# rapidsai/cudf

Measured on AMD Instinct MI355X. Metric: rows/sec + achieved HBM GB/s: 1e9-row int64 sort & hash-join, 1/2/4/8 GPU, higher is better.
Workload: dtype int64; 1 GPU; 1e+09-row int64 radix sort (cudf::sort, keys only); rows_per_gpu=1000000000, algo=0, parallelism=1 GPU

## Files before the change

cudf_amd/csrc/gx_common.hpp:

```cpp
#pragma once

#include <hip/hip_runtime.h>

#include <atomic>
#include <stdint.h>

#include "../../include/cudf_amd/gx.h"
#include "gx_lds_book.hpp"

#define GX_WAVE 64

#define GX_HIP_TRY(expr)                           \
  do {                                             \
    const int _e = (int)(expr);                    \
    if (_e != (int)hipSuccess) return _e;          \
  } while (0)

#define GX_LAUNCH_CHECK()                          \
  do {                                             \
    hipError_t _e = hipGetLastError();             \
    if (_e != hipSuccess) return (int)_e;          \
  } while (0)

namespace gx {
// ... 47 lines not shown
template <typename Kernel, typename... Args>
inline int launch_lds(const Device& dev, Kernel kernel, dim3 grid, dim3 block, size_t lds_bytes, hipStream_t s, Args&&... args)
{
  GX_HIP_TRY(lds_book().ensure(reinterpret_cast<const void*>(kernel), dev.id, (int)lds_bytes, set_max_dynamic_lds));
  hipLaunchKernelGGL(kernel, grid, block, lds_bytes, s, static_cast<Args&&>(args)...);
  return 0;
}
inline int max_resident_wgs(const Device& dev, const void* kernel, int block, size_t lds_bytes, int* wgs)
{
  GX_HIP_TRY(lds_book().ensure(kernel, dev.id, (int)lds_bytes, set_max_dynamic_lds));
  GX_HIP_TRY(hipOccupancyMaxActiveBlocksPerMultiprocessor(wgs, kernel, block, lds_bytes));
  if (*wgs < 1) *wgs = 1;
  return 0;
}

__device__ __forceinline__ unsigned lane_id()
{
  return __builtin_amdgcn_mbcnt_hi(~0u, __builtin_amdgcn_mbcnt_lo(~0u, 0u));
}
__device__ __forceinline__ uint64_t lanemask_lt() { return (1ull << lane_id()) - 1ull; }
__device__ __forceinline__ uint64_t ballot(bool p) { return __builtin_amdgcn_ballot_w64(p); }

template <typename T, typename F>
__device__ __forceinline__ T shfl_words(T v, F f)
{
  static_assert(sizeof(T) % 4 == 0, "shuffle payload must be a multiple of 4 bytes");
  uint32_t w[sizeof(T) / 4];
  __builtin_memcpy(w, &v, sizeof(T));
#pragma unroll
  for (unsigned k = 0; k < sizeof(T) / 4; ++k) w[k] = f(w[k]);
  T r;
  __builtin_memcpy(&r, w, sizeof(T));
  return r;
}
template <typename T>
__device__ __forceinline__ T shfl_up(T v, unsigned delta)
{
  return shfl_words(v, [delta](uint32_t x) { return (uint32_t)__shfl_up((int)x, delta, GX_WAVE); });
}
template <typename T>
__device__ __forceinline__ T shfl(T v, int src)
{
  return shfl_words(v, [src](uint32_t x) { return (uint32_t)__shfl((int)x, src, GX_WAVE); });
}
template <typename T>
__device__ __forceinline__ T shfl_xor(T v, int m)
{
  return shfl_words(v, [m](uint32_t x) { return (uint32_t)__shfl_xor((int)x, m, GX_WAVE); });
}

template <int NBITS>
__device__ __forceinline__ void match_rank(uint32_t d, bool live, uint64_t active, uint32_t& lower, uint32_t& count)
{
  uint32_t m_lo = (uint32_t)active, m_hi = (uint32_t)(active >> 32);
#pragma unroll
  for (int b = 0; b < NBITS; ++b) {
    const int beta   = __builtin_amdgcn_sbfe(d, b, 1);
    const uint64_t v = ballot(live && beta != 0);
    m_lo             = __builtin_amdgcn_bitop3_b32(m_lo, (uint32_t)v, (uint32_t)beta, 0x90);
    m_hi             = __builtin_amdgcn_bitop3_b32(m_hi, (uint32_t)(v >> 32), (uint32_t)beta, 0x90);
  }
  lower = __builtin_amdgcn_mbcnt_hi(m_hi, __builtin_amdgcn_mbcnt_lo(m_lo, 0u));
  count = (uint32_t)__builtin_popcount(m_lo) + (uint32_t)__builtin_popcount(m_hi);
}

template <int NBITS>
__device__ __forceinline__ uint32_t lds_rank_few(uint32_t* counters, uint32_t d, bool live)
{
  const uint64_t active = ballot(live);
  uint32_t m_lo = (uint32_t)active, m_hi = (uint32_t)(active >> 32);
#pragma unroll
  for (int b = 0; b < NBITS; ++b) {
    const int beta   = __builtin_amdgcn_sbfe(d, b, 1);
    const uint64_t v = ballot(live && beta != 0);
    m_lo             = __builtin_amdgcn_bitop3_b32(m_lo, (uint32_t)v, (uint32_t)beta, 0x90);
    m_hi             = __builtin_amdgcn_bitop3_b32(m_hi, (uint32_t)(v >> 32), (uint32_t)beta, 0x90);
  }
  const uint32_t lower = __builtin_amdgcn_mbcnt_hi(m_hi, __builtin_amdgcn_mbcnt_lo(m_lo, 0u));
  const uint32_t count = (uint32_t)__builtin_popcount(m_lo) + (uint32_t)__builtin_popcount(m_hi);
  const uint64_t m     = ((uint64_t)m_hi << 32) | m_lo;
  const int leader     = m ? __builtin_ctzll(m) : (int)lane_id();
  uint32_t base        = 0;
  if (live && lower == 0) base = atomicAdd(&counters[d], count);
  base = (uint32_t)__builtin_amdgcn_ds_bpermute(leader << 2, (int)base);
  return live ? base + lower : 0u;
}

__device__ __forceinline__ void match_rank8(uint32_t d, bool live, uint64_t active, uint32_t& lower, uint32_t& count)
{
  match_rank<8>(d, live, active, lower, count);
}

template <int M>
__device__ __forceinline__ uint32_t lane_xor32(uint32_t v)
{
  if constexpr (M == 1) return (uint32_t)__builtin_amdgcn_update_dpp(0, (int)v, 0xB1, 0xF, 0xF, false);
  else if constexpr (M == 2) return (uint32_t)__builtin_amdgcn_update_dpp(0, (int)v, 0x4E, 0xF, 0xF, false);
  else if constexpr (M == 3) return (uint32_t)__builtin_amdgcn_update_dpp(0, (int)v, 0x1B, 0xF, 0xF, false);
  else if constexpr (M == 7) return (uint32_t)__builtin_amdgcn_update_dpp(0, (int)v, 0x141, 0xF, 0xF, false);
  else if constexpr (M == 15) return (uint32_t)__builtin_amdgcn_update_dpp(0, (int)v, 0x140, 0xF, 0xF, false);
  else return (uint32_t)__builtin_amdgcn_ds_bpermute((int)((lane_id() ^ (unsigned)M) << 2), (int)v);
}
template <int M>
__device__ __forceinline__ uint64_t lane_xor64(uint64_t v)
{
  return ((uint64_t)lane_xor32<M>((uint32_t)(v >> 32)) << 32) | lane_xor32<M>((uint32_t)v);
}
template <int M, int LOWBIT>
__device__ __forceinline__ void cmpx(uint64_t& k)
{
  const uint64_t o   = lane_xor64<M>(k);
  const bool keepmin = (lane_id() & (unsigned)LOWBIT) == 0;
  k                  = ((k < o) == keepmin) ? k : o;
}
__device__ __forceinline__ void wave_bitonic64(uint64_t& k)
{
  cmpx<1, 1>(k);
  cmpx<3, 2>(k); cmpx<1, 1>(k);
  cmpx<7, 4>(k); cmpx<2, 2>(k); cmpx<1, 1>(k);
  cmpx<15, 8>(k); cmpx<4, 4>(k); cmpx<2, 2>(k); cmpx<1, 1>(k);
  cmpx<31, 16>(k); cmpx<8, 8>(k); cmpx<4, 4>(k); cmpx<2, 2>(k); cmpx<1, 1>(k);
  cmpx<63, 32>(k); cmpx<16, 16>(k); cmpx<8, 8>(k); cmpx<4, 4>(k); cmpx<2, 2>(k); cmpx<1, 1>(k);
}
__device__ __forceinline__ void wave_halfclean64(uint64_t& k)
{
  cmpx<32, 32>(k); cmpx<16, 16>(k); cmpx<8, 8>(k); cmpx<4, 4>(k); cmpx<2, 2>(k); cmpx<1, 1>(k);
}
__device__ __forceinline__ void wave_bitonic128(uint64_t& k0, uint64_t& k1)
{
  wave_bitonic64(k0);
  wave_bitonic64(k1);
  const uint64_t o1 = lane_xor64<63>(k1), o0 = lane_xor64<63>(k0);
  k0 = k0 < o1 ? k0 : o1;
  k1 = k1 < o0 ? o0 : k1;
  wave_halfclean64(k0);
  wave_halfclean64(k1);
}

__device__ __forceinline__ uint32_t lds_rank(uint32_t* counters, uint32_t d, bool live)
{
  const uint64_t act = ballot(live);
  if (act == 0) return 0;
  const int leader    = __builtin_ctzll(act);
  const uint32_t dl   = shfl(d, leader);
  const uint64_t same = ballot(live && d == dl);
  if (same == act || __builtin_popcountll(same) >= 8) {
    uint32_t base = 0;
    if ((int)lane_id() == leader) base = atomicAdd(&counters[dl], (uint32_t)__builtin_popcountll(same));
    base = shfl(base, leader);
    if (live && d == dl) return base + (uint32_t)__builtin_popcountll(same & lanemask_lt());
    return live ? atomicAdd(&counters[d], 1u) : 0u;
  }
  return live ? atomicAdd(&counters[d], 1u) : 0u;
}

struct SumOp {
  template <typename T>
  __device__ __forceinline__ T operator()(T a, T b) const { return a + b; }
};
struct MinOp {
  template <typename T>
  __device__ __forceinline__ T operator()(T a, T b) const { return b < a ? b : a; }
};
struct MaxOp {
  template <typename T>
  __device__ __forceinline__ T operator()(T a, T b) const { return a < b ? b : a; }
};
struct ProdOp {
  template <typename T>
  __device__ __forceinline__ T operator()(T a, T b) const { return a * b; }
};

template <int CTRL, int RM, typename T>
__device__ __forceinline__ T dpp_take(T v)
{
  return shfl_words(v, [](uint32_t x) { return (uint32_t)__builtin_amdgcn_update_dpp((int)x, (int)x, CTRL, RM, 0xF, false); });
}
template <int SRC, typename T>
__device__ __forceinline__ T read_lane(T v)
{
  return shfl_words(v, [](uint32_t x) { return (uint32_t)__builtin_amdgcn_readlane((int)x, SRC); });
}
template <typename T, typename Op>
__device__ __forceinline__ T wave_inclusive_scan(T v, Op op)
{
  const unsigned l = lane_id();
  { const T o = dpp_take<0x111, 0xF>(v); if ((l & 15u) >= 1u) v = op(o, v); }
  { const T o = dpp_take<0x112, 0xF>(v); if ((l & 15u) >= 2u) v = op(o, v); }
  { const T o = dpp_take<0x114, 0xF>(v); if ((l & 15u) >= 4u) v = op(o, v); }
  { const T o = dpp_take<0x118, 0xF>(v); if ((l & 15u) >= 8u) v = op(o, v); }
  { const T o = dpp_take<0x142, 0xA>(v); if (l & 16u) v = op(o, v); }
  { const T o = dpp_take<0x143, 0xC>(v); if (l >= 32u) v = op(o, v); }
  return v;
}

template <typename T, typename Op>
__device__ __forceinline__ T wave_reduce(T v, Op op)
{
#pragma unroll
  for (int d = GX_WAVE / 2; d >= 1; d >>= 1) v = op(v, shfl_xor(v, d));
  return v;
}

template <int BT, typename T, typename Op>
__device__ __forceinline__ T block_exclusive_scan(T v, T identity, Op op, T* lds, T* total)
{
  constexpr int NW = BT / GX_WAVE;
  const unsigned l = lane_id();
  const unsigned w = threadIdx.x / GX_WAVE;
  T inc            = wave_inclusive_scan(v, op);
  if (l == GX_WAVE - 1) lds[w] = inc;
  __syncthreads();
  if (w == 0) {
    T x = (l < NW) ? lds[l] : identity;
    T s = wave_inclusive_scan(x, op);
    if (l < NW) lds[l] = s;
  }
  __syncthreads();
  T wave_prefix = (w == 0) ? identity : lds[w - 1];
  T exc         = shfl_up(inc, 1);
  if (l == 0) exc = identity;
  if (total) *total = lds[NW - 1];
  T r = op(wave_prefix, exc);
  __syncthreads();
  return r;
}

__device__ __forceinline__ uint64_t dpp_wave_shl1_u64(uint64_t v, uint64_t fill)
{
  const int lo = __builtin_amdgcn_update_dpp((int)(uint32_t)fill, (int)(uint32_t)v, 0x130, 0xF, 0xF, false);
  const int hi = __builtin_amdgcn_update_dpp((int)(uint32_t)(fill >> 32), (int)(uint32_t)(v >> 32), 0x130, 0xF, 0xF, false);
  return ((uint64_t)(uint32_t)hi << 32) | (uint32_t)lo;
}
__device__ __forceinline__ uint64_t dpp_wave_shr1_u64(uint64_t v, uint64_t fill)
{
  const int lo = __builtin_amdgcn_update_dpp((int)(uint32_t)fill, (int)(uint32_t)v, 0x138, 0xF, 0xF, false);
  const int hi = __builtin_amdgcn_update_dpp((int)(uint32_t)(fill >> 32), (int)(uint32_t)(v >> 32), 0x138, 0xF, 0xF, false);
  return ((uint64_t)(uint32_t)hi << 32) | (uint32_t)lo;
}
__device__ __forceinline__ bool wave_split_sort(uint64_t* keys, uint32_t cnt, uint32_t* cw ,
                                                int sh, uint64_t& k0, uint64_t& k1)
{
  const unsigned lane = lane_id();
  const uint32_t e0 = 2 * lane, e1 = 2 * lane + 1;
  k0 = e0 < cnt ? keys[e0] : ~0ull;
  k1 = e1 < cnt ? keys[e1] : ~0ull;
  uint4* cw4  = reinterpret_cast<uint4*>(cw);
  cw4[lane]   = make_uint4(0u, 0u, 0u, 0u);
  const uint32_t b0 = (uint32_t)(k0 >> sh) & 0xFFu, b1 = (uint32_t)(k1 >> sh) & 0xFFu;
  const uint32_t r0 = e0 < cnt ? atomicAdd(&cw[b0], 1u) : 0u;
  const uint32_t r1 = e1 < cnt ? atomicAdd(&cw[b1], 1u) : 0u;
  uint4 c = cw4[lane];
  uint32_t mx = c.x > c.y ? c.x : c.y;
  mx          = c.z > mx ? c.z : mx;
  mx          = c.w > mx ? c.w : mx;
  if (ballot(mx > 4u) != 0) return false;
  const uint32_t sum = c.x + c.y + c.z + c.w;
  const uint32_t inc = wave_inclusive_scan(sum, SumOp());
  uint32_t run       = inc - sum;
  uint4 st;
  st.x = run; run += c.x;
  st.y = run; run += c.y;
  st.z = run; run += c.z;
  st.w = run;
  cw4[lane] = st;
  if (e0 < cnt) keys[cw[b0] + r0] = k0;
  if (e1 < cnt) keys[cw[b1] + r1] = k1;
  k0 = e0 < cnt ? keys[e0] : ~0ull;
  k1 = e1 < cnt ? keys[e1] : ~0ull;
#pragma unroll
  for (int ph = 0; ph < 2; ++ph) {
    {
      const bool sw     = k1 < k0;
      const uint64_t lo = sw ? k1 : k0, hi = sw ? k0 : k1;
      k0 = lo;
      k1 = hi;
    }
    {
      const uint64_t nxt = dpp_wave_shl1_u64(k0, ~0ull);
      const uint64_t prv = dpp_wave_shr1_u64(k1, 0ull);
      k1                 = nxt < k1 ? nxt : k1;
      k0                 = prv > k0 ? prv : k0;
    }
  }
  return true;
}

__device__ __forceinline__ uint32_t wave_inclusive_sum_dpp(uint32_t v)
{
  v += (uint32_t)__builtin_amdgcn_update_dpp(0, (int)v, 0x111, 0xF, 0xF, false);
  v += (uint32_t)__builtin_amdgcn_update_dpp(0, (int)v, 0x112, 0xF, 0xF, false);
  v += (uint32_t)__builtin_amdgcn_update_dpp(0, (int)v, 0x114, 0xF, 0xF, false);
  v += (uint32_t)__builtin_amdgcn_update_dpp(0, (int)v, 0x118, 0xF, 0xF, false);
  v += (uint32_t)__builtin_amdgcn_update_dpp(0, (int)v, 0x142, 0xA, 0xF, false);
  v += (uint32_t)__builtin_amdgcn_update_dpp(0, (int)v, 0x143, 0xC, 0xF, false);
  return v;
}

__device__ __forceinline__ unsigned wave_split_sort_x2(uint64_t* keysA, uint32_t cntA, uint64_t* keysB, uint32_t cntB,
                                                       uint32_t* cw , int sh, uint64_t& a0,
                                                       uint64_t& a1, uint64_t& b0, uint64_t& b1)
{
  const unsigned lane = lane_id();
  const uint32_t e0 = 2 * lane, e1 = 2 * lane + 1;
  uint32_t* cwA = cw;
  uint32_t* cwB = cw + 128;
// ... 233 lines not shown
```

cudf_amd/csrc/gx_sort.hip:

```cpp
#include "gx_common.hpp"
#include <cstdlib>
#include <type_traits>
#include <vector>
#include "gx_scan.hpp"

namespace gx {
namespace sort {

constexpr int BINS       = 256;
constexpr int MAX_PASSES = 8;
constexpr int BT         = 512;
constexpr int NW         = BT / GX_WAVE;
constexpr int NRANGE     = 8;

constexpr int CS_MAXBITS = 15;
constexpr int NB2MAX     = 1024;
constexpr int NB9        = 512;

struct HybridPlan {
  int32_t attempt;
  int32_t ok;
  int32_t shift0;
  int32_t shift2, bits2;
  int32_t nlocal;
// ... 700 lines not shown
#pragma unroll
          for (int k = 0; k < LBW; ++k) {
            const int64_t q = p - k;
            v[k]            = (q >= 0) ? load_agent_u64(&a.status[q * BINS + tid]) : pack_status(2u, epoch, 0u);
          }
#pragma unroll
          for (int k = 0; k < LBW; ++k) {
            if (!done) {
              unsigned long long x = v[k];
              uint32_t spins       = 0;
              unsigned long long spin_t0 = 0;
              while ((x >> 62) == 0 || ((unsigned)(x >> 32) & 0xFFu) != epoch) {
                if (spin_guard(spins, spin_t0, plan, a.spin_ticks)) {
                  x = pack_status(2u, epoch, 0u);
                  break;
                }
                __builtin_amdgcn_s_sleep(2);
                x = load_agent_u64(&a.status[(p - k) * BINS + tid]);
              }
              prefix += (uint32_t)x;
              if ((x >> 62) == 2u) done = true;
            }
          }
          p -= LBW;
        }
        if (tile != a.inject_tile) store_agent_u64(&a.status[tile * BINS + tid], pack_status(2u, epoch, prefix + pub_count));
      }
      gbase = plan->gbin[pass][tid] + prefix;
    } else {
      gbase = a.tile_off[(int64_t)tid * a_ntiles + tile];
    }
    s_gdelta[tid] = gbase - bin_start;
  }
  __syncthreads();

#pragma unroll
  for (int j = 0; j < KPT; ++j) {
    const int i = j * BT + (int)tid;
    if (i < nvalid) {
      const KeyT k       = s_keys[i];
      const uint32_t d   = (uint32_t)(to_sortable<KeyT, KIND>(k, desc_mask) >> shift) & 0xFFu;
      const uint32_t dst = s_gdelta[d] + (uint32_t)i;
      kout[dst]          = k;
      if (HAS_VAL) vout[dst] = s_vals[i];
    }
  }
  if (MULTI) __syncthreads();
  }
}

template <typename KeyT, int KIND, int KPT>
__global__ void __launch_bounds__(BT) k_tile_hist(PassArgs a, uint32_t* tile_hist)
{
  constexpr int TILE = BT * KPT;
  __shared__ uint32_t s_hist[BINS];
  SortPlan* plan = a.plan;
  const int pass = a.pass;
  if (plan->pass_skip[pass]) return;
  const KeyT* kin      = static_cast<const KeyT*>(a.kbuf[plan->pass_src[pass]]);
  const KeyT desc_mask = (KeyT)a.desc_mask;
  const int shift      = pass * 8;
  const unsigned tid   = threadIdx.x;
  if (tid < BINS) s_hist[tid] = 0;
  __syncthreads();
  const int64_t tile = xcd_swizzle(blockIdx.x, gridDim.x);
  const int64_t base = tile * TILE;
  const int nvalid   = (int)((a.n - base < (int64_t)TILE) ? (a.n - base) : (int64_t)TILE);
  const unsigned lane = lane_id();
#pragma unroll
  for (int j = 0; j < KPT; ++j) {
    const int i = j * BT + (int)tid;
    if (i < nvalid) {
      const uint32_t d      = (uint32_t)(to_sortable<KeyT, KIND>(kin[base + i], desc_mask) >> shift) & 0xFFu;
      const uint64_t active = ballot(true);
      const uint32_t d0     = __builtin_amdgcn_readfirstlane(d);
      if (ballot(d == d0) == active) {
        if ((int)lane == __builtin_ctzll(active)) atomicAdd(&s_hist[d0], (uint32_t)__builtin_popcountll(active));
      } else {
        atomicAdd(&s_hist[d], 1u);
      }
    }
  }
  __syncthreads();
  if (tid < BINS) tile_hist[(int64_t)tid * a.ntiles + tile] = s_hist[tid];
}

template <typename KeyT, bool HAS_VAL>
__global__ void __launch_bounds__(256) k_finalize_copy(PassArgs a)
{
  if (a.plan->num_active != 0) return;
  const bool mode_b    = a.plan->hy.lsd_mode != 0;
  const KeyT* kin      = static_cast<const KeyT*>(mode_b ? a.kbufB[0] : a.kbuf[0]);
  KeyT* kout           = static_cast<KeyT*>(mode_b ? a.kbufB[1] : a.kbuf[1]);
  const int64_t a_n    = mode_b ? (int64_t)a.plan->hy.lsd_n : a.n;
  const int64_t stride = (int64_t)gridDim.x * blockDim.x;
  for (int64_t i = (int64_t)blockIdx.x * blockDim.x + threadIdx.x; i < a_n; i += stride) {
    kout[i] = kin[i];
    if (HAS_VAL) a.vbuf[1][i] = a.vbuf[0] ? a.vbuf[0][i] : (uint32_t)i;
  }
}

template <typename KeyT, bool HAS_VAL>
__global__ void __launch_bounds__(256) k_reverse_nan_block(KeyT* keys, uint32_t* vals, int64_t n)
{
  constexpr KeyT SIGN = KeyT(1) << (sizeof(KeyT) * 8 - 1);
  constexpr KeyT EXP  = (sizeof(KeyT) == 8) ? KeyT(0x7FF0000000000000ull) : KeyT(0x7F800000u);
  __shared__ long long s_cnt;
  if (threadIdx.x == 0) {
    int64_t lo = 0, hi = n;
    while (lo < hi) {
      const int64_t mid = lo + (hi - lo) / 2;
      if ((keys[mid] & KeyT(~SIGN)) > EXP) lo = mid + 1; else hi = mid;
    }
    s_cnt = lo;
  }
  __syncthreads();
  const int64_t cnt    = s_cnt;
  const int64_t half   = cnt / 2;
  const int64_t stride = (int64_t)gridDim.x * blockDim.x;
  for (int64_t i = (int64_t)blockIdx.x * blockDim.x + threadIdx.x; i < half; i += stride) {
    const int64_t j = cnt - 1 - i;
    const KeyT a = keys[i], b = keys[j];
    keys[i] = b;
    keys[j] = a;
    if (HAS_VAL) {
      const uint32_t va = vals[i], vb2 = vals[j];
      vals[i] = vb2;
      vals[j] = va;
    }
  }
}

__device__ __forceinline__ unsigned xcc_id() { return __builtin_amdgcn_s_getreg(20 | (0 << 6) | (3 << 11)) & 7u; }

struct MsdArgs {
  const void* in;
  void* out;
  const uint32_t* vin;
  uint32_t* vout;
  SortPlan* plan;
  unsigned long long* status;
  const uint32_t* base;
  uint32_t* cellcount;
  uint32_t cellcap;
  int64_t n;
  int level;
  int exp;
  uint64_t desc_mask;
  unsigned long long spin_ticks = 0;
  long long inject_tile         = -1;
};

template <typename KeyT, int KIND, bool HAS_VAL, int KPT, int LBW, int NBL>
__global__ void __launch_bounds__(BT, (KPT <= 8 ? 8 : (KPT <= 12 ? 6 : 4))) k_msd_pass(MsdArgs a)
{
  constexpr int TILE = BT * KPT;
  constexpr int NB   = 1 << NBL;
  static_assert(NB <= BT, "one thread per bin");
  constexpr bool STABLE = KIND == K_FLOAT || HAS_VAL;
  constexpr int WROWS   = STABLE ? NW : 2;
  extern __shared__ __attribute__((aligned(16))) char smem[];
  KeyT* s_keys       = reinterpret_cast<KeyT*>(smem);
  uint32_t* s_vals   = reinterpret_cast<uint32_t*>(smem + (size_t)TILE * sizeof(KeyT));
  constexpr bool HIST16 = STABLE && HAS_VAL && NBL == 9;
  using HistT           = typename std::conditional<HIST16, uint16_t, uint32_t>::type;
  uint32_t* s_whist  = s_vals + (HAS_VAL ? TILE : 0);
  HistT* s_whist16   = reinterpret_cast<HistT*>(s_whist);
  uint32_t* s_gdelta = s_whist + (HIST16 ? WROWS * NB / 2 : WROWS * NB);
  uint32_t* s_limit  = s_gdelta + NB;
  uint32_t* s_scan   = s_limit + NB;
  uint32_t* s_misc   = s_scan + 16;

  SortPlan* plan = a.plan;
  HybridPlan& hy = plan->hy;
  const int lvl  = a.level;
  if (!hy.attempt || plan->hf.state == 3) return;
  const KeyT* kin      = static_cast<const KeyT*>(a.in);
  KeyT* kout           = static_cast<KeyT*>(a.out);
  const uint32_t* vin  = a.vin;
  uint32_t* vout       = a.vout;
  const KeyT desc_mask = (KeyT)a.desc_mask;
  const uint32_t dmask = lvl == 0 ? 0xFFu : ((1u << hy.bits2) - 1u);
  const Digit0 dig     = lvl == 0 ? digit0_of(hy, (int)(8 * sizeof(KeyT))) : Digit0{hy.shift2, 0, dmask, 0u};
  const int nseg       = lvl == 0 ? NRANGE : BINS;
  const unsigned tid   = threadIdx.x;
  const unsigned lane  = lane_id();
  const unsigned w     = tid / GX_WAVE;
  const unsigned epoch = 9u + (unsigned)lvl;

  if (tid == 0) {
    const unsigned x = ((a.exp & 1) && lvl == 1) ? 0u : ((a.exp & 2) ? (blockIdx.x % NRANGE) : xcc_id());
    uint32_t g       = 0xFFFFFFFFu;
    for (int i = 0; i < NRANGE; ++i) {
      const unsigned y   = (x + i) % NRANGE;
      const uint32_t ntl = hy.list_tile0[lvl][y + 1] - hy.list_tile0[lvl][y];
      if (ntl == 0) continue;
      const uint32_t t = atomicAdd(&plan->cnt.ctr[lvl][y].v, 1u);
      if (t < ntl) {
        g = hy.list_tile0[lvl][y] + t;
        break;
      }
    }
    s_misc[0] = g;
  }
  __syncthreads();
  {
    const uint32_t g = s_misc[0];
    if (g != 0xFFFFFFFFu && (int)tid < nseg) {
      const uint32_t lo = hy.seg_tile0[lvl][tid], hi = hy.seg_tile0[lvl][tid + 1];
      if (lo <= g && g < hi) {
        s_misc[1] = tid;
        s_misc[2] = g - lo;
      }
    }
  }
  __syncthreads();
  const uint32_t gtile = s_misc[0];
  if (gtile == 0xFFFFFFFFu) return;
  const uint32_t seg   = s_misc[1];
  const uint32_t jt    = s_misc[2];
  const int64_t base   = (int64_t)hy.seg_start[lvl][seg] + (int64_t)jt * TILE;
  const int64_t remain = (int64_t)hy.seg_count[lvl][seg] - (int64_t)jt * TILE;
  const int nvalid     = (int)(remain < (int64_t)TILE ? remain : (int64_t)TILE);
  const uint32_t l1cap  = lvl == 1 ? cell_cap(hy, seg) : 0u;
  const uint32_t l1base = lvl == 1 ? cell_slot(hy, seg, 0u) : 0u;

  KeyT key[KPT];
  uint32_t val[HAS_VAL ? KPT : 1];
  const int wbase = (int)w * (KPT * GX_WAVE) + (int)lane;
  if (nvalid == TILE) {
#pragma unroll
    for (int j = 0; j < KPT; ++j) key[j] = kin[base + wbase + j * GX_WAVE];
  } else {
#pragma unroll
    for (int j = 0; j < KPT; ++j) {
      const int idx = wbase + j * GX_WAVE;
      key[j]        = (idx < nvalid) ? kin[base + idx] : KeyT(0);
    }
  }
  if (HAS_VAL) {
#pragma unroll
    for (int j = 0; j < KPT; ++j) {
      const int idx = wbase + j * GX_WAVE;
      val[j]        = (idx < nvalid) ? (vin ? vin[base + idx] : (uint32_t)(base + idx)) : 0u;
    }
  }
  HistT* my_hist = s_whist16 + w * NB;
  uint32_t packed[KPT];
  uint32_t tile_count = 0;
  if (STABLE) {
#pragma unroll
    for (int k = 0; k < NB / ((HIST16 ? 2 : 1) * GX_WAVE); ++k) reinterpret_cast<uint32_t*>(my_hist)[lane + k * GX_WAVE] = 0;
#pragma unroll
    for (int j = 0; j < KPT; ++j) {
      const int idx = wbase + j * GX_WAVE;
      uint32_t d    = dig(to_sortable<KeyT, KIND>(key[j], desc_mask));
      if (idx >= nvalid) d = NB - 1;
      uint32_t lower, cnt;
      match_rank<NBL>(d, true, ~0ull, lower, cnt);
      const uint32_t prev = my_hist[d];
      if (lower == 0) my_hist[d] = (HistT)(prev + cnt);
      packed[j] = (d << 16) | (prev + lower);
    }
    __syncthreads();
    if (tid < NB) {
      uint32_t sum = 0;
#pragma unroll
      for (int w2 = 0; w2 < NW; ++w2) {
        const uint32_t c         = s_whist16[w2 * NB + tid];
        s_whist16[w2 * NB + tid] = (HistT)sum;
        sum += c;
      }
      tile_count = sum;
    }
  } else {
    if (tid < NB) s_whist[tid] = 0;
    __syncthreads();
#pragma unroll
    for (int j = 0; j < KPT; ++j) {
      const int idx    = wbase + j * GX_WAVE;
      const uint32_t d = dig(to_sortable<KeyT, KIND>(key[j], desc_mask));
      const uint32_t r = lds_rank(s_whist, d, idx < nvalid);
      packed[j]        = (d << 16) | r;
    }
    __syncthreads();
    if (tid < NB) tile_count = s_whist[tid];
  }
  uint32_t pub_count = tile_count;
  if (STABLE && tid == NB - 1) pub_count -= (uint32_t)(TILE - nvalid);
  if (tid < NB) {
    if ((long long)gtile != a.inject_tile) store_agent_u64(&a.status[(int64_t)gtile * NB + tid], pack_status(jt == 0 ? 2u : 1u, epoch, pub_count));
  }
  const uint32_t bin_start = block_exclusive_scan<BT>(tile_count, 0u, SumOp(), s_scan, (uint32_t*)nullptr);
  if (tid < NB) {
    if (STABLE) {
#pragma unroll
      for (int w2 = 0; w2 < NW; ++w2) s_whist16[w2 * NB + tid] = (HistT)(s_whist16[w2 * NB + tid] + bin_start);
    } else {
      s_whist[NB + tid] = bin_start;
    }
  }
  __syncthreads();

#pragma unroll
  for (int j = 0; j < KPT; ++j) {
    const uint32_t d = packed[j] >> 16;
    if (STABLE) {
      const uint32_t pos = (uint32_t)my_hist[d] + (packed[j] & 0xFFFFu);
      s_keys[pos]        = key[j];
      if (HAS_VAL) s_vals[pos] = val[j];
    } else if (wbase + j * GX_WAVE < nvalid) {
      s_keys[s_whist[NB + d] + (packed[j] & 0xFFFFu)] = key[j];
    }
  }

  if (tid < NB) {
    uint32_t prefix = 0;
    if (jt > 0) {
      int64_t p = (int64_t)gtile - 1;
      bool done = false;
      while (!done) {
        unsigned long long v[LBW];
#pragma unroll
        for (int k = 0; k < LBW; ++k) {
          const int64_t q = p - k;
          v[k]            = (q >= 0) ? load_agent_u64(&a.status[q * NB + tid]) : pack_status(2u, epoch, 0u);
        }
#pragma unroll
        for (int k = 0; k < LBW; ++k) {
          if (!done) {
            unsigned long long x = v[k];
            uint32_t spins       = 0;
            unsigned long long spin_t0 = 0;
            while ((x >> 62) == 0 || ((unsigned)(x >> 32) & 0xFFu) != epoch) {
              if (spin_guard(spins, spin_t0, a.plan, a.spin_ticks)) {
                x = pack_status(2u, epoch, 0u);
                break;
              }
              __builtin_amdgcn_s_sleep(2);
              x = load_agent_u64(&a.status[(p - k) * NB + tid]);
            }
            prefix += (uint32_t)x;
            if ((x >> 62) == 2u) done = true;
          }
        }
        p -= LBW;
      }
      if ((long long)gtile != a.inject_tile) store_agent_u64(&a.status[(int64_t)gtile * NB + tid], pack_status(2u, epoch, prefix + pub_count));
    }
    uint32_t gb, lim = 0xFFFFFFFFu;
    if (lvl == 0) {
      gb = a.base[seg * NB2MAX + tid];
    } else {
      const bool live = tid < (1u << hy.bits2);
      const uint32_t cellcap = l1cap;
      gb              = live ? l1base + tid * l1cap : 0u;
      lim             = live ? gb + cellcap : 0u;
      if (live) {
        if (prefix + pub_count > cellcap && !__hip_atomic_load(&hy.overflow, __ATOMIC_RELAXED, __HIP_MEMORY_SCOPE_AGENT))
          atomicExch(&hy.overflow, 1);
        if (gtile + 1 == hy.seg_tile0[1][seg + 1]) a.cellcount[seg * NB2MAX + tid] = prefix + pub_count;
      }
    }
    s_limit[tid]  = lim;
    s_gdelta[tid] = gb + prefix - bin_start;
  }
  __syncthreads();

#pragma unroll
  for (int j = 0; j < KPT; ++j) {
    const int i = j * BT + (int)tid;
    if (i < nvalid) {
      const KeyT k       = s_keys[i];
      const uint32_t d   = dig(to_sortable<KeyT, KIND>(k, desc_mask));
      const uint32_t dst = s_gdelta[d] + (uint32_t)i;
      if (dst < s_limit[d]) {
        kout[dst] = k;
        if (HAS_VAL) vout[dst] = s_vals[i];
      }
    }
  }
}

__global__ void __launch_bounds__(GX_WAVE) k_plan2(SortPlan* plan, uint32_t* __restrict__ cellcount,
                                                   uint32_t* __restrict__ cellstart, int npass, int cursor_path)
{
  HybridPlan& hy = plan->hy;
  if (!hy.attempt || (plan->hf.state == 3) != (cursor_path != 0)) return;
  constexpr int PER    = NB2MAX / GX_WAVE;
  const int b          = blockIdx.x;
  const unsigned lane  = lane_id();
  const uint32_t start = hy.gbin0[b];
  const uint32_t count = hy.hist0[b];
  const int nb2        = 1 << hy.bits2;
  const bool eqb = cursor_path && plan->sp.on && plan->sp.eq[b];
  const bool nrb = cursor_path && plan->sp.on && sp_narrow(plan->sp, (uint32_t)b, hy.bits2);
  uint32_t c[PER], sum = 0, mx = 0;
#pragma unroll
  for (int k = 0; k < PER; ++k) {
    const int d2 = (int)lane * PER + k;
    c[k]         = d2 < nb2 ? cellcount[b * NB2MAX + d2] : 0u;
    sum += c[k];
    if (eqb) {
      if (d2 == 0) cellcount[b * NB2MAX] = 0u;
      c[k] = 0u;
    }
    if (nrb && d2 < nb2) cellcount[b * NB2MAX + d2] = 0u;
    if (!nrb) mx = c[k] > mx ? c[k] : mx;
  }
  const uint32_t inc = wave_inclusive_sum_dpp(sum);
  uint32_t run       = start + inc - sum;
#pragma unroll
  for (int k = 0; k < PER; ++k) {
    const int d2 = (int)lane * PER + k;
    if (d2 < nb2) cellstart[b * NB2MAX + d2] = run;
    run += c[k];
  }
  const uint32_t total = shfl(inc, GX_WAVE - 1);
  mx                   = wave_reduce(mx, MaxOp());
  if (mx > cell_cap(hy, (uint32_t)b) && lane == 0) atomicExch(&hy.overflow, 1);
  if (cursor_path && !nrb) {
    uint32_t bc = 0, bk = 0;
#pragma unroll
    for (int k = 0; k < PER; ++k) {
      if (c[k] > cell_cap(hy, (uint32_t)b)) {
        ++bc;
        bk += c[k];
      }
    }
    bc = wave_reduce(bc, SumOp());
    bk = wave_reduce(bk, SumOp());
    if (lane == 0) {
      hy.bigcnt[b]  = bc;
      hy.bigkeys[b] = bk;
    }
  }
  if (lane == 0) {
    atomicMax(&hy.max_cell, mx);
    if (total != count) atomicExch(&hy.bad, 1);
    __threadfence();
    if (atomicAdd(&hy.plan2_done, 1u) == (uint32_t)BINS - 1u) {
      const int overflow     = atomicAdd(&hy.overflow, 0);
      const int bad          = (cursor_path || !overflow) && atomicAdd(&hy.bad, 0);
      const uint32_t maxcell = atomicMax(&hy.max_cell, 0u);
      if (bad) atomicCAS(&plan->status, 0, 3);
      const int big = (overflow || maxcell > (uint32_t)hy.cell_max) ? 1 : 0;
      const int ok = (!bad && (cursor_path || !big)) ? 1 : 0;
      hy.ok        = ok;
      hy.big       = (ok && big) ? 1 : 0;
      if (ok && !big) {
        for (int p = 0; p < npass; ++p) plan->pass_skip[p] = 1;
        plan->num_active = -1;
      }
    }
  }
}


template <typename KeyT, int KIND, bool HAS_VAL, int CL2>
__device__ __forceinline__ void pairs_write_out(KeyT* s_keys, const KeyT* __restrict__ in_cell, KeyT* __restrict__ out,
                                                const uint32_t* __restrict__ vin_cell, uint32_t* __restrict__ vout,
                                                int64_t start, uint32_t m, int shift2, KeyT desc_mask, bool write_keys = true,
                                                bool padded = false)
{
  const KeyT* in      = in_cell - start;
  const uint32_t* vin = vin_cell ? vin_cell - start : nullptr;
  constexpr int LS_KPT = 16, LS_BT = (1 << CL2) / LS_KPT, LS_POS_BITS = CL2;
  const unsigned tid = threadIdx.x;
  const KeyT lowmask = (KeyT(1) << shift2) - KeyT(1);
  const KeyT hi      = to_sortable<KeyT, KIND>(in[start], desc_mask) & ~lowmask;
  uint32_t pos[LS_KPT];
#pragma unroll
  for (int j = 0; j < LS_KPT; ++j) {
    const int i = j * LS_BT + (int)tid;
    pos[j]      = 0;
    if ((uint32_t)i < m) {
      const KeyT wd = s_keys[padded ? i + (i >> 4) : i];
      pos[j]        = (uint32_t)wd & ((1u << LS_POS_BITS) - 1u);
      if (KIND != K_FLOAT && write_keys) out[start + i] = to_sortable<KeyT, KIND>(hi | ((wd >> LS_POS_BITS) & lowmask), desc_mask);
    }
  }
  __syncthreads();
  if (KIND == K_FLOAT && write_keys) {
#pragma unroll
    for (int j = 0; j < LS_KPT; ++j) {
      const int i = j * LS_BT + (int)tid;
      if ((uint32_t)i < m) s_keys[i] = in[start + i];
    }
    __syncthreads();
#pragma unroll
    for (int j = 0; j < LS_KPT; ++j) {
      const int i = j * LS_BT + (int)tid;
      if ((uint32_t)i < m) out[start + i] = s_keys[pos[j]];
    }
    __syncthreads();
  }
  if (!HAS_VAL) return;
  uint32_t* s_idx = reinterpret_cast<uint32_t*>(s_keys);
#pragma unroll
  for (int j = 0; j < LS_KPT; ++j) {
    const int i = j * LS_BT + (int)tid;
    if ((uint32_t)i < m) s_idx[i] = vin[start + i];
  }
  __syncthreads();
#pragma unroll
  for (int j = 0; j < LS_KPT; ++j) {
    const int i = j * LS_BT + (int)tid;
    if ((uint32_t)i < m) vout[start + i] = s_idx[pos[j]];
  }
}

template <typename KeyT, int KIND, bool HAS_VAL, int CL2>
__device__ __forceinline__ bool place_applies(const HybridPlan& hy, int exp)
{
  constexpr bool PACKED = HAS_VAL || KIND == K_FLOAT;
  const int word_bits   = hy.shift2 + (PACKED ? CL2 : 0);
  return hy.nlocal > 0 && !(exp & (32 | 16 | 8 | 4)) && word_bits >= CL2 && word_bits <= 64;
}
template <typename KeyT, int KIND, bool HAS_VAL>
struct PlaceWord {
  typedef typename std::conditional<sizeof(KeyT) == 8 || HAS_VAL || KIND == K_FLOAT, uint64_t, uint32_t>::type type;
};
constexpr size_t place_lds_bytes(int cl2, int word_bytes = 8)
{
  return (size_t)((1 << cl2) + (1 << cl2) / 16) * word_bytes + (size_t)(1 << cl2) + (size_t)((1 << cl2) / 16) * 4 + 32 * 4;
}

struct CellMeta {
  uint32_t m, cap, slot, start;
};
__device__ __forceinline__ CellMeta cell_meta(const HybridPlan& hy, const uint32_t* __restrict__ hist2, const uint32_t* __restrict__ base2, uint32_t cell)
{
  const uint32_t b = cell >> hy.bits2, d2 = cell & ((1u << hy.bits2) - 1u);
// ... 312 lines not shown
      };
      for (int sb = (int)w; sb < NSB; sb += 2 * LS_NW) {
        if (exp & 4) break;
        const int sbB       = sb + LS_NW;
        const uint32_t cntA = s_cnt[sb], oA = s_start[sb];
        const uint32_t cntB = sbB < NSB ? s_cnt[sbB] : 0u, oB = sbB < NSB ? s_start[sbB] : 0u;
        const bool doA = cntA > 1, doB = cntB > 1;
        if (!doA && !doB) continue;
        KeyT* subA = s_keys + oA;
        KeyT* subB = s_keys + oB;
        unsigned okm = 0;
        uint64_t a0 = 0, a1 = 0, b0 = 0, b1 = 0;
        if (sshift >= 8 && !(exp & 16))
          okm = wave_split_sort_x2(reinterpret_cast<uint64_t*>(subA), doA ? cntA : 0u, reinterpret_cast<uint64_t*>(subB),
                                   doB ? cntB : 0u, my_hist, sshift - 8, a0, a1, b0, b1);
        if (okm & 1u) emit2(subA, cntA, oA, a0, a1);
        else if (doA) network(subA, cntA, oA);
        if (okm & 2u) emit2(subB, cntB, oB, b0, b1);
        else if (doB) network(subB, cntB, oB);
      }
      if (!PAIRS) {
        if (!(exp & 4)) {
          if (tid < NSB && s_cnt[tid] == 1) out[start + s_start[tid]] = unsort(s_keys[s_start[tid]]);
          return;
        }
      }
      __syncthreads();
      if constexpr (!NARROW) {
        if (PAIRS) {
          pairs_write_out<KeyT, KIND, HAS_VAL, CL2>(s_keys, in + start, out, HAS_VAL ? vin + start : nullptr, vout, start, m, hy.shift2, desc_mask_in, !(exp & 64));
          return;
        }
      }
#pragma unroll
      for (int j = 0; j < LS_KPT; ++j) {
        const int i = j * LS_BT + (int)tid;
        if ((uint32_t)i < m) out[start + i] = unsort(s_keys[i]);
      }
      return;
    }
#pragma unroll
    for (int j = 0; j < LS_KPT; ++j) {
      if constexpr (NARROW) key[j] = key[j];
      else key[j] = PAIRS ? key[j] : from_sortable<KeyT, IK>(key[j], desc_mask);
    }
    __syncthreads();
  }
  for (int lp = 0; lp < nlocal; ++lp) {
    const int shift      = hy.lshift[lp] + pos_shift;
    const uint32_t dmask = (1u << hy.lbits[lp]) - 1u;
#pragma unroll
    for (int k = 0; k < BINS / GX_WAVE; ++k) my_hist[lane + k * GX_WAVE] = 0;
    uint32_t packed[LS_KPT];
#pragma unroll
    for (int j = 0; j < LS_KPT; ++j) {
      const int idx     = wbase + j * GX_WAVE;
      const bool live   = (uint32_t)idx < m;
      const uint64_t act = ballot(live);
      packed[j]         = 0;
      if (act == 0) continue;
      const uint32_t d = (uint32_t)(sortable(key[j]) >> shift) & dmask;
      uint32_t lower, cnt;
      match_rank8(d, live, act, lower, cnt);
      if (live) {
        const uint32_t prev = my_hist[d];
        if (lower == 0) my_hist[d] = prev + cnt;
        packed[j] = (d << 16) | (prev + lower);
      }
    }
    __syncthreads();
    uint32_t tile_count = 0;
    if (tid < BINS) {
      uint32_t sum = 0;
#pragma unroll
      for (int w2 = 0; w2 < LS_NW; ++w2) {
        const uint32_t c         = s_whist[w2 * BINS + tid];
        s_whist[w2 * BINS + tid] = sum;
        sum += c;
      }
      tile_count = sum;
    }
    const uint32_t bin_start = block_exclusive_scan<LS_BT>(tile_count, 0u, SumOp(), s_scan, (uint32_t*)nullptr);
    if (tid < BINS) {
#pragma unroll
      for (int w2 = 0; w2 < LS_NW; ++w2) s_whist[w2 * BINS + tid] += bin_start;
    }
    __syncthreads();
#pragma unroll
    for (int j = 0; j < LS_KPT; ++j) {
      const int idx = wbase + j * GX_WAVE;
      if ((uint32_t)idx < m) s_keys[my_hist[packed[j] >> 16] + (packed[j] & 0xFFFFu)] = key[j];
    }
    __syncthreads();
    if (lp + 1 < nlocal) {
#pragma unroll
      for (int j = 0; j < LS_KPT; ++j) {
        const int idx = wbase + j * GX_WAVE;
        key[j]        = ((uint32_t)idx < m) ? s_keys[idx] : KeyT(0);
      }
      __syncthreads();
    }
  }
  if (nlocal == 0) {
#pragma unroll
    for (int j = 0; j < LS_KPT; ++j) {
      const int idx = wbase + j * GX_WAVE;
      if ((uint32_t)idx < m) {
        if (PAIRS) {
          out[start + idx] = in[start + idx];
          if (HAS_VAL) vout[start + idx] = vin[start + idx];
        } else {
          out[start + idx] = put(key[j]);
        }
      }
    }
    return;
  }
  if constexpr (!NARROW) {
    if (PAIRS) {
      pairs_write_out<KeyT, KIND, HAS_VAL, CL2>(s_keys, in + start, out, HAS_VAL ? vin + start : nullptr, vout, start, m, hy.shift2, desc_mask_in, !(exp & 64));
      return;
    }
  }
#pragma unroll
  for (int j = 0; j < LS_KPT; ++j) {
    const int i = j * LS_BT + (int)tid;
    if ((uint32_t)i < m) out[start + i] = put(s_keys[i]);
  }
}


template <typename KeyT, int KIND, bool HAS_VAL, int CL2, typename IoT = KeyT>
__global__ void __launch_bounds__((1 << CL2) / 16, 4) k_local_sort(const IoT* in, IoT* __restrict__ out,
                                                      const uint32_t* vin, uint32_t* __restrict__ vout,
                                                      KeyT desc_mask_in, SortPlan* plan,
                                                      const uint32_t* __restrict__ hist2, const uint32_t* __restrict__ base2,
                                                      int exp = 0, int cursor_path = 0, const uint32_t* __restrict__ todo = nullptr)
{
  HybridPlan& hy = plan->hy;
  if (!hy.attempt || !hy.ok || (plan->hf.state == 3) != (cursor_path != 0)) return;
  if (hy.cell_max != (1 << CL2)) return;
  const bool listed    = todo != nullptr && place_applies<IoT, KIND, HAS_VAL, CL2>(hy, exp);
  const uint32_t count = listed ? hy.todo_count : ((uint32_t)BINS << hy.bits2);
  for (uint32_t e = blockIdx.x; e < count; e += gridDim.x) {
    local_sort_cell<KeyT, KIND, HAS_VAL, CL2, IoT>(listed ? todo[e] : e, in, out, vin, vout, desc_mask_in, plan, hist2, base2, exp);
    __syncthreads();
  }
}

constexpr int HF_CHUNK = GX_WAVE;

template <typename KeyT, int KIND, bool HIST>
__global__ void __launch_bounds__(256) k_hf_sample(const KeyT* __restrict__ in, int64_t n, KeyT desc_mask, SortPlan* plan, int stride,
                                                   int64_t range_rows)
{
  HybridPlan& hy = plan->hy;
  FastPlan& hf   = plan->hf;
  if (HIST && (hf.state != 1 || hf.hist_ready)) return;
  __shared__ uint32_t s_hist[NRANGE * BINS];
  __shared__ unsigned long long s_red[2 * 4];
  const unsigned tid = threadIdx.x, lane = lane_id();
  for (int i = tid; i < NRANGE * BINS; i += 256) s_hist[i] = 0;
  __syncthreads();
  const Digit0 dig      = HIST ? digit0_of(hy, (int)(8 * sizeof(KeyT))) : Digit0{(int)(8 * sizeof(KeyT) - 8), 0, 0xFFu, 0u};
  const int64_t step    = (int64_t)stride * HF_CHUNK;
  const int64_t nchunks = div_up(n, step);
  const int64_t nw      = (int64_t)gridDim.x * 4;
  constexpr int U       = 8;
  KeyT vor = 0, vnor = 0, vfold = 0;
  for (int64_t c0 = (int64_t)blockIdx.x * 4 + tid / GX_WAVE; c0 < nchunks; c0 += nw * U) {
    KeyT raw[U];
#pragma unroll
    for (int u = 0; u < U; ++u) {
      const int64_t row = (c0 + u * nw) * step + lane;
      raw[u]            = (c0 + u * nw < nchunks && row < n) ? in[row] : KeyT(0);
    }
#pragma unroll
    for (int u = 0; u < U; ++u) {
      const int64_t row = (c0 + u * nw) * step + lane;
      const bool live   = c0 + u * nw < nchunks && row < n;
      const KeyT k      = to_sortable<KeyT, KIND>(raw[u], desc_mask);
      if (!HIST && live) {
        if constexpr (KIND == K_FTOTAL) {
          if (float_unclean<KeyT>(raw[u])) hf.fail = 1;
        }
        vor |= k;
        vnor |= (KeyT)~k;
        if (KIND == K_SIGNED) vfold |= (KeyT)(raw[u] ^ (KeyT)(KeyT(0) - (KeyT)(raw[u] >> (8 * sizeof(KeyT) - 1))));
      }
      const int64_t r64 = range_rows > 0 ? row / range_rows : (int64_t)(NRANGE - 1);
      const int r       = r64 < NRANGE - 1 ? (int)r64 : NRANGE - 1;
      (void)lds_rank(s_hist + r * BINS, dig(k), live);
    }
  }
  if (!HIST) {
    const unsigned long long wo = wave_reduce((unsigned long long)vor, [](unsigned long long x, unsigned long long y) { return x | y; });
    const unsigned long long wn = wave_reduce((unsigned long long)vnor, [](unsigned long long x, unsigned long long y) { return x | y; });
    if (lane == 0) {
      s_red[tid / GX_WAVE]     = wo;
      s_red[4 + tid / GX_WAVE] = wn;
    }
    __syncthreads();
    if (tid == 0) {
      atomicOr(&hy.or_mask, s_red[0] | s_red[1] | s_red[2] | s_red[3]);
      atomicOr(&hy.nor_mask, s_red[4] | s_red[5] | s_red[6] | s_red[7]);
    }
    if (KIND == K_SIGNED) {
      const unsigned long long wf = wave_reduce((unsigned long long)vfold, [](unsigned long long x, unsigned long long y) { return x | y; });
      if (lane == 0 && wf) atomicOr(&hy.fold_x, wf);
    }
  }
  __syncthreads();
  for (int i = tid; i < NRANGE * BINS; i += 256) {
    const uint32_t c = s_hist[i];
    if (c) atomicAdd(&hf.samp[i / BINS][i % BINS], c);
  }
}

__device__ __forceinline__ int64_t hf_range_rows(int r, int64_t n, int64_t range_rows)
{
  const int64_t b = (int64_t)r * range_rows < n ? (int64_t)r * range_rows : n;
  const int64_t e = (r == NRANGE - 1) ? n : (b + range_rows < n ? b + range_rows : n);
  return e - b;
}

__device__ __forceinline__ void hf_give_up(SortPlan* plan, int state)
{
  plan->hy.attempt  = 0;
  plan->hy.or_mask  = 0;
  plan->hy.nor_mask = 0;
  plan->hy.overflow = 0;
  plan->hy.fold     = 0;
  plan->hy.fold_x   = 0;
  plan->hf.state    = state;
}

__global__ void __launch_bounds__(BINS) k_hf_plan(SortPlan* plan, int stage, int key_bits, int64_t n, int bits2, int cell_max, int stride,
                                                  int64_t range_rows, int tile_rows, unsigned long long slot_rows, float margin, int min_shift2,
                                                  int bits2_max, unsigned long long cell_budget = 0, int signed_keys = 0, int allow_counting = 0,
                                                  int allow_split = 0)
{
  __shared__ uint32_t s_tmp[BINS / GX_WAVE + 1];
  HybridPlan& hy = plan->hy;
  FastPlan& hf   = plan->hf;
  const int t    = threadIdx.x;
  if (stage == 0) {
    if (hf.fail) {
      if (t == 0) hf_give_up(plan, 0);
      return;
    }
    const unsigned long long V = hy.or_mask & hy.nor_mask;
    const int fh               = signed_keys ? fold_height(hy.fold_x, V, key_bits) : 0;
    const int top              = fh ? fh : (V ? 63 - __builtin_clzll(V) : 0);
    const int shift0           = top - 7;
    const int shift2           = shift0 - bits2;
    if (V == 0 || shift2 < min_shift2) {
      if (t == 0) {
        const int cs_top = V ? 63 - __builtin_clzll(V) : 0;
        const bool cs    = allow_counting && V != 0 && cs_top < CS_MAXBITS;
        const unsigned long long ormask = hy.or_mask;
        hf_give_up(plan, V == 0 ? 0 : (cs ? 5 : 4));
        if (cs) {
          hf.cs_bits = cs_top + 1;
          hf.cs_base = ormask & ~((1ull << (cs_top + 1)) - 1ull);
        }
      }
      return;
    }
    const bool spec_ok = shift0 == key_bits - 8;
    if (!spec_ok) {
      for (int r = 0; r < NRANGE; ++r) hf.samp[r][t] = 0;
    }
    if (t == 0) {
      hf.hist_ready = spec_ok ? 1 : 0;
      hy.attempt   = 1;
      hy.fold      = fh ? 1 : 0;
      hy.shift0    = shift0;
      hy.bits2     = bits2;
      hy.shift2    = shift2;
      hy.cell_max  = cell_max;
      hy.need_hist = 0;
      hf.stride    = stride;
      hf.state     = 1;
    }
    return;
  }
  if (hf.state != 1) return;
  SplitPlan& sp = plan->sp;
  if (stage == 1) {
    if (hf.slots_ready) return;
    if (sp.req < 0) {
      if (t == 0) hf_give_up(plan, 4);
      return;
    }
    uint32_t cap[NRANGE];
    uint32_t sum = 0;
    for (int r = 0; r < NRANGE; ++r) {
      const uint32_t c = hf.samp[r][t];
      uint32_t total;
      (void)block_exclusive_scan<BINS>(c, 0u, SumOp(), s_tmp, &total);
      const int64_t rows = hf_range_rows(r, n, range_rows);
      const double scale = total ? (double)rows / (double)total : 0.0;
      double cp          = (double)c * scale + (double)margin * scale * __builtin_sqrt((double)c + 1.0) + 2.0 * stride * HF_CHUNK + 64.0;
      if (cp > (double)rows) cp = (double)rows;
      if (cp < 0.0) cp = 0.0;
      cap[r] = ((uint32_t)cp + 15u) & ~15u;
      sum += cap[r];
    }
    uint32_t total;
    uint32_t run = block_exclusive_scan<BINS>(sum, 0u, SumOp(), s_tmp, &total);
    if ((unsigned long long)total > slot_rows) {
      if (t == 0) hf_give_up(plan, 0);
      return;
    }
    {
      double est = 0.0;
      for (int r = 0; r < NRANGE; ++r) {
        uint32_t tot_r;
        (void)block_exclusive_scan<BINS>(hf.samp[r][t], 0u, SumOp(), s_tmp, &tot_r);
        if (tot_r) est += (double)hf.samp[r][t] * ((double)hf_range_rows(r, n, range_rows) / (double)tot_r);
      }
      const double fits  = (double)((1ull << bits2_max) - 1ull) * (double)cell_max;
      const double over  = est > 2.0 * (fits + (double)cell_max) ? est : (est > fits + (double)cell_max ? est - fits : 0.0);
      const uint32_t o32 = (uint32_t)(over < 4.0e9 ? over : 4.0e9);
      uint32_t osum;
      (void)block_exclusive_scan<BINS>(o32 >> 4, 0u, SumOp(), s_tmp, &osum);
      if (!sp.on && allow_split && !sp.req && (double)osum * 16.0 > 0.03 * (double)n) {
        for (int r = 0; r < NRANGE; ++r) hf.samp[r][t] = 0;
        if (t == 0) sp.req = 1;
        return;
      }
      if (!sp.on && (double)osum * 16.0 > 0.75 * (double)n) {
        if (t == 0) hf_give_up(plan, 4);
        return;
      }
    }
    for (int r = 0; r < NRANGE; ++r) {
      hf.slot0[r][t] = run;
      hf.cap0[r][t]  = cap[r];
      run += cap[r];
    }
    if (sp.on) {
      uint32_t m[SP_NPIECE];
      uint32_t M = 0;
#pragma unroll
// ... 592 lines not shown
      nz_val[g]   = b;
      ++g;
      run += c;
    }
  }
  if (threadIdx.x == 0) {
    nz_start[groups] = total;
    hf.cs_groups     = groups;
    for (int p = 0; p < npass; ++p) plan->pass_skip[p] = 1;
    plan->num_active = -1;
    __threadfence();
    plan->hy.ok = 1;
  }
}

template <typename KeyT, int KIND>
__global__ void __launch_bounds__(256) k_cs_fill(KeyT* __restrict__ out, int64_t n, KeyT desc_mask, const SortPlan* plan,
                                                 const uint32_t* __restrict__ nz_start, const uint32_t* __restrict__ nz_val)
{
  const FastPlan& hf = plan->hf;
  if (hf.state != 5 || !plan->hy.ok) return;
  __shared__ uint32_t s_start[CS_TILE + 2];
  __shared__ uint32_t s_g[2];
  const uint32_t groups = hf.cs_groups;
  const KeyT base       = (KeyT)hf.cs_base;
  const int64_t tiles   = div_up(n, (int64_t)CS_TILE);
  for (int64_t tile = blockIdx.x; tile < tiles; tile += gridDim.x) {
    const uint32_t lo = (uint32_t)(tile * CS_TILE);
    const uint32_t hi = (uint32_t)((tile + 1) * CS_TILE < n ? (tile + 1) * CS_TILE : n);
    if (threadIdx.x < 2) {
      const uint32_t pos = threadIdx.x == 0 ? lo : hi - 1;
      uint32_t a = 0, b = groups;
      while (b - a > 1) {
        const uint32_t mid = (a + b) >> 1;
        if (nz_start[mid] <= pos) a = mid; else b = mid;
      }
      s_g[threadIdx.x] = a;
    }
    __syncthreads();
    const uint32_t g0 = s_g[0], g1 = s_g[1];
    if (g0 == g1) {
      const KeyT v = from_sortable<KeyT, KIND>((KeyT)(base | (KeyT)nz_val[g0]), desc_mask);
      for (uint32_t i = lo + threadIdx.x; i < hi; i += 256) __builtin_nontemporal_store(v, &out[i]);
    } else {
      const uint32_t ng = g1 - g0 + 1;
      for (uint32_t k = threadIdx.x; k < ng; k += 256) s_start[k] = nz_start[g0 + k];
      __syncthreads();
      for (uint32_t i = lo + threadIdx.x; i < hi; i += 256) {
        uint32_t a = 0, b = ng;
        while (b - a > 1) {
          const uint32_t mid = (a + b) >> 1;
          if (s_start[mid] <= i) a = mid; else b = mid;
        }
        __builtin_nontemporal_store(from_sortable<KeyT, KIND>((KeyT)(base | (KeyT)nz_val[g0 + a]), desc_mask), &out[i]);
      }
    }
    __syncthreads();
  }
}

__global__ void __launch_bounds__(256) k_hf_clear_status(const SortPlan* plan, uint4* __restrict__ status, size_t n16)
{
  if ((plan->hf.state == 3 || plan->hf.state == 5) && plan->hy.ok && !plan->hy.lsd_mode) return;
  const size_t stride = (size_t)gridDim.x * 256;
  for (size_t i = (size_t)blockIdx.x * 256 + threadIdx.x; i < n16; i += stride) status[i] = uint4{0u, 0u, 0u, 0u};
}

constexpr int BIG_LIST = 1 << 16;
__global__ void __launch_bounds__(BINS) k_big_plan(SortPlan* plan, unsigned long long xcap)
{
  HybridPlan& hy = plan->hy;
  if (plan->hf.state != 3 || !hy.ok || !hy.big) return;
  __shared__ uint32_t s_tmp[BINS / GX_WAVE + 1];
  const int b = threadIdx.x;
  uint32_t nbig, xtotal;
  const uint32_t k0 = block_exclusive_scan<BINS>(hy.bigcnt[b], 0u, SumOp(), s_tmp, &nbig);
  const uint32_t x0 = block_exclusive_scan<BINS>(hy.bigkeys[b], 0u, SumOp(), s_tmp, &xtotal);
  if (nbig == 0 || nbig > (uint32_t)BIG_LIST || (unsigned long long)xtotal > xcap) {
    if (b == 0) {
      hy.ok  = 0;
      hy.big = 0;
    }
    return;
  }
  hy.biglist0[b]  = k0;
  hy.bigx0[b]     = x0;
  hy.bigbucket[b] = hy.bigcnt[b] ? 1u : 0u;
  if (b == 0) {
    hy.nbig     = nbig;
    hy.lsd_n    = xtotal;
    hy.lsd_mode = 1;
  }
}
__global__ void __launch_bounds__(GX_WAVE) k_big_cells(const SortPlan* plan, const uint32_t* __restrict__ cellcount, uint32_t* __restrict__ xoff,
                                                       uint32_t* __restrict__ biglist)
{
  const HybridPlan& hy = plan->hy;
  const int b = blockIdx.x;
  if (!(hy.ok && hy.lsd_mode) || !hy.bigbucket[b]) return;
  constexpr int PER   = NB2MAX / GX_WAVE;
  const unsigned lane = lane_id();
  const int nb2       = 1 << hy.bits2;
  const uint32_t cap  = cell_cap(hy, (uint32_t)b);
  uint32_t c[PER], cnt = 0, keys = 0;
#pragma unroll
  for (int k = 0; k < PER; ++k) {
    const int d2 = (int)lane * PER + k;
    c[k]         = d2 < nb2 ? cellcount[b * NB2MAX + d2] : 0u;
    if (c[k] > cap) {
      ++cnt;
      keys += c[k];
    }
  }
  uint32_t kk = hy.biglist0[b] + wave_inclusive_sum_dpp(cnt) - cnt;
  uint32_t x  = hy.bigx0[b] + wave_inclusive_sum_dpp(keys) - keys;
#pragma unroll
  for (int k = 0; k < PER; ++k) {
    if (c[k] > cap) {
      const uint32_t idx  = (uint32_t)(b * NB2MAX + (int)lane * PER + k);
      xoff[idx]           = x;
      biglist[2 * kk]     = idx;
      biglist[2 * kk + 1] = x;
      ++kk;
      x += c[k];
    }
  }
}

template <typename KeyT>
__global__ void __launch_bounds__(256) k_big_distribute(const SortPlan* plan, const KeyT* __restrict__ xsorted, KeyT* __restrict__ out,
                                                        const uint32_t* __restrict__ biglist, const uint32_t* __restrict__ cellstart)
{
  const HybridPlan& hy = plan->hy;
  if (!(hy.ok && hy.lsd_mode)) return;
  const uint32_t n = (uint32_t)hy.lsd_n, nbig = hy.nbig;
  const uint32_t stride = gridDim.x * 256u;
  for (uint32_t i = blockIdx.x * 256u + threadIdx.x; i < n; i += stride) {
    uint32_t lo = 0, hi = nbig;
    while (hi - lo > 1) {
      const uint32_t mid = (lo + hi) >> 1;
      if (biglist[2 * mid + 1] <= i) lo = mid; else hi = mid;
    }
    out[cellstart[biglist[2 * lo]] + (i - biglist[2 * lo + 1])] = xsorted[i];
  }
}

template <typename KeyT>
constexpr int hf_kpt()
{
  return sizeof(KeyT) == 8 ? 16 : 24;
}

template <typename KeyT, int KIND, int LVL, int NBL>
__global__ void __launch_bounds__(BT, 4) k_hf_scatter(const KeyT* __restrict__ in, KeyT* __restrict__ out, KeyT desc_mask, SortPlan* plan,
                                                     uint32_t* __restrict__ cellcur, uint32_t cellcap, int64_t n, KeyT* __restrict__ fin = nullptr)
{
  constexpr int KPT = hf_kpt<KeyT>(), TILE = BT * KPT, NB = 1 << NBL, BPT = NB > BT ? NB / BT : 1;
  extern __shared__ __attribute__((aligned(16))) char smem[];
  KeyT* s_keys      = reinterpret_cast<KeyT*>(smem);
  uint32_t* s_cnt   = reinterpret_cast<uint32_t*>(smem + (size_t)TILE * sizeof(KeyT));
  uint32_t* s_delta = s_cnt + NB;
  uint32_t* s_limit = s_delta + NB;
  uint32_t* s_scan  = s_limit + NB;
  uint32_t* s_misc  = s_scan + 16;
  unsigned long long* s_red = reinterpret_cast<unsigned long long*>(s_misc + 4);
  __shared__ uint2 s_wt[(LVL >= 1 && sizeof(KeyT) == 8) ? SP_NPIECE : 1];
  HybridPlan& hy = plan->hy;
  FastPlan& hf   = plan->hf;
  if (hf.state != (LVL == 0 ? 1 : 3)) return;
  if (LVL == 0 && plan->sp.on) return;
  if (LVL == 2 && !(hy.ok && hy.lsd_mode)) return;
  const bool split     = LVL >= 1 && sizeof(KeyT) == 8 && plan->sp.on;
  const uint32_t* xoff = cellcur + 2 * BINS * NB2MAX;
  uint32_t* rescur     = cellcur + 3 * BINS * NB2MAX;
  const unsigned tid = threadIdx.x;
  const int64_t v    = xcd_swizzle((int64_t)blockIdx.x, (int64_t)gridDim.x);
  int64_t base;
  int nvalid;
  uint32_t seg;
  if (LVL == 0) {
    const int64_t per = (int64_t)gridDim.x / NRANGE;
    seg               = (per > 0 && v / per < NRANGE - 1) ? (uint32_t)(v / per) : (uint32_t)(NRANGE - 1);
    base              = v * TILE;
    nvalid            = (int)(n - base < (int64_t)TILE ? n - base : (int64_t)TILE);
  } else if (!hf.ext) {
    if (v >= (int64_t)hf.reg_tile0[BINS * NRANGE]) return;
    constexpr int QPT = BINS * NRANGE / BT;
#pragma unroll
    for (int k = 0; k < QPT; ++k) {
      const int q       = (int)tid * QPT + k;
      const uint32_t lo = hf.reg_tile0[q], hi = hf.reg_tile0[q + 1];
      if ((int64_t)lo <= v && v < (int64_t)hi) {
        s_misc[0] = (uint32_t)q;
        s_misc[1] = (uint32_t)(v - lo);
      }
    }
    __syncthreads();
    const uint32_t q  = s_misc[0];
    const uint32_t jt = s_misc[1];
    seg               = q / NRANGE;
    if (LVL == 2 && !hy.bigbucket[seg]) return;
    base              = (int64_t)hf.reg_start[q] + (int64_t)jt * TILE;
    const int64_t rem = (int64_t)hf.reg_count[q] - (int64_t)jt * TILE;
    nvalid            = (int)(rem < (int64_t)TILE ? rem : (int64_t)TILE);
  } else {
    const uint32_t nreg    = hf.nreg;
    const uint32_t* rtile0 = hf.x_tile0;
    if (v >= (int64_t)rtile0[nreg]) return;
    for (uint32_t q = tid; q < nreg; q += BT) {
      const uint32_t lo = rtile0[q], hi = rtile0[q + 1];
      if ((int64_t)lo <= v && v < (int64_t)hi) {
        s_misc[0] = q;
        s_misc[1] = (uint32_t)(v - lo);
      }
    }
    __syncthreads();
    const uint32_t q  = s_misc[0];
    const uint32_t jt = s_misc[1];
    seg               = hf.x_bucket[q];
    if (LVL == 2 && !hy.bigbucket[seg]) return;
    base              = (int64_t)hf.x_start[q] + (int64_t)jt * TILE;
    const int64_t rem = (int64_t)hf.x_count[q] - (int64_t)jt * TILE;
    nvalid            = (int)(rem < (int64_t)TILE ? rem : (int64_t)TILE);
  }
  const uint32_t dmask = LVL == 0 ? 0xFFu : ((1u << hy.bits2) - 1u);
  const Digit0 dig     = LVL == 0 ? digit0_of(hy, (int)(8 * sizeof(KeyT))) : Digit0{hy.shift2, 0, dmask, 0u};
  const uint32_t cap_s  = LVL >= 1 ? cell_cap(hy, seg) : 0u;
  const uint32_t base_s = LVL >= 1 ? cell_slot(hy, seg, 0u) : 0u;
  SpCell spc{0ull, 1ull, 0u, 63};
  if (split) {
    if (plan->sp.eq[seg]) {
      if (LVL == 2) return;
      if (tid == 0) s_misc[2] = atomicAdd(&cellcur[seg * NB2MAX], (uint32_t)nvalid);
      __syncthreads();
      const int64_t dst0 = (int64_t)hy.gbin0[seg] + (int64_t)s_misc[2];
#pragma unroll
      for (int j = 0; j < KPT; ++j) {
        const int idx = j * BT + (int)tid;
        if (idx < nvalid) fin[dst0 + idx] = in[base + idx];
      }
      return;
    }
    spc = sp_cell_of(plan->sp, seg);
    if (tid < (unsigned)SP_NPIECE) s_wt[tid] = plan->sp.wt[seg][tid];
  }
  const uint32_t spnc = split ? plan->sp.nc[seg] : 1u;
  auto spdig          = [&](KeyT k) -> uint32_t {
    if constexpr (sizeof(KeyT) == 8) return sp_cell(sp_warp(sp_frac(spc, (unsigned long long)k), s_wt), spnc);
    else return dig(k);
  };
  if (split && sp_narrow(plan->sp, seg, hy.bits2)) {
    if (LVL == 2) return;
    for (int b = tid; b < NB; b += BT) s_cnt[b] = 0;
    __syncthreads();
#pragma unroll
    for (int j = 0; j < KPT; ++j) {
      const int idx   = j * BT + (int)tid;
      const bool live = idx < nvalid;
      const KeyT k    = to_sortable<KeyT, KIND>(in[base + (live ? idx : 0)], desc_mask);
      (void)lds_rank(s_cnt, spdig(k), live);
    }
    __syncthreads();
    for (int b = tid; b < NB; b += BT) {
      const uint32_t c = s_cnt[b];
      if (c) atomicAdd(&cellcur[seg * NB2MAX + b], c);
    }
    return;
  }

  KeyT key[KPT];
  if (nvalid == TILE) {
#pragma unroll
    for (int j = 0; j < KPT; ++j) key[j] = in[base + j * BT + (int)tid];
  } else {
#pragma unroll
    for (int j = 0; j < KPT; ++j) {
      const int idx = j * BT + (int)tid;
      key[j]        = in[base + (idx < nvalid ? idx : 0)];
    }
  }
  for (int b = tid; b < NB; b += BT) s_cnt[b] = 0;
  if constexpr (LVL == 0 && KIND == K_FTOTAL) {
    bool unclean = false;
#pragma unroll
    for (int j = 0; j < KPT; ++j) unclean |= float_unclean<KeyT>(key[j]);
    if (unclean) hf.fail = 1;
  }
  if (LVL == 0) {
    auto mform = [&](KeyT k) -> KeyT {
      if constexpr (KIND == K_FTOTAL) return to_sortable<KeyT, KIND>(k, KeyT(0));
      else return k;
    };
    KeyT vor = mform(key[0]), vnor = (KeyT)~mform(key[0]);
#pragma unroll
    for (int j = 1; j < KPT; ++j) {
      vor |= mform(key[j]);
      vnor |= (KeyT)~mform(key[j]);
    }
    const unsigned long long wo = wave_reduce((unsigned long long)vor, [](unsigned long long x, unsigned long long y) { return x | y; });
    const unsigned long long wn = wave_reduce((unsigned long long)vnor, [](unsigned long long x, unsigned long long y) { return x | y; });
    if (lane_id() == 0) {
      s_red[tid / GX_WAVE]      = wo;
      s_red[NW + tid / GX_WAVE] = wn;
    }
    if (KIND == K_SIGNED && hy.fold) {
      KeyT vf = 0;
#pragma unroll
      for (int j = 0; j < KPT; ++j) vf |= (KeyT)(key[j] ^ (KeyT)(KeyT(0) - (KeyT)(key[j] >> (8 * sizeof(KeyT) - 1))));
      const unsigned long long wf = wave_reduce((unsigned long long)vf, [](unsigned long long x, unsigned long long y) { return x | y; });
      if (lane_id() == 0 && (wf & ~__hip_atomic_load(&hy.fold_x, __ATOMIC_RELAXED, __HIP_MEMORY_SCOPE_AGENT))) atomicOr(&hy.fold_x, wf);
    }
  }
  __syncthreads();
  if (LVL == 0 && tid == 0) {
    unsigned long long o = 0, no = 0;
    for (int k = 0; k < NW; ++k) {
      o |= s_red[k];
      no |= s_red[NW + k];
    }
    if (o & ~__hip_atomic_load(&hy.or_mask, __ATOMIC_RELAXED, __HIP_MEMORY_SCOPE_AGENT)) atomicOr(&hy.or_mask, o);
    if (no & ~__hip_atomic_load(&hy.nor_mask, __ATOMIC_RELAXED, __HIP_MEMORY_SCOPE_AGENT)) atomicOr(&hy.nor_mask, no);
  }
  constexpr bool RANK16 = sizeof(KeyT) == 4;
  uint32_t packed[RANK16 ? KPT / 2 : KPT];
  if constexpr (RANK16) {
#pragma unroll
    for (int j = 0; j < KPT / 2; ++j) packed[j] = 0;
  }
  auto rank_all = [&](auto&& digf) {
#pragma unroll
    for (int j = 0; j < KPT; ++j) {
      const bool live  = j * BT + (int)tid < nvalid;
      const KeyT k     = to_sortable<KeyT, KIND>(key[j], desc_mask);
      const uint32_t d = digf(k);
      const uint32_t r = lds_rank(s_cnt, d, live);
      if constexpr (RANK16) packed[j >> 1] |= r << (16 * (j & 1));
      else packed[j] = (d << 16) | r;
    }
  };
  if (split) rank_all(spdig); else rank_all(dig);
  __syncthreads();
  uint32_t c[BPT], g[BPT], sbase[BPT], scap[BPT];
  bool skip[BPT];
  uint32_t csum = 0;
#pragma unroll
  for (int k = 0; k < BPT; ++k) {
    const uint32_t bin = tid * BPT + k;
    c[k] = g[k] = sbase[k] = scap[k] = 0;
    skip[k] = false;
    if (bin < (uint32_t)NB) {
      c[k] = s_cnt[bin];
      if (LVL == 0) {
        sbase[k] = hf.slot0[seg][bin];
        scap[k]  = hf.cap0[seg][bin];
        if (c[k]) g[k] = atomicAdd(&hf.cur0[seg][bin], c[k]);
      } else if (LVL == 1 && bin <= dmask) {
        sbase[k] = base_s + bin * cap_s;
        scap[k]  = cap_s;
        if (c[k]) g[k] = atomicAdd(&cellcur[seg * NB2MAX + bin], c[k]);
      } else if (LVL == 2 && bin <= dmask) {
        const uint32_t total = cellcur[seg * NB2MAX + bin];
        if (total > cap_s) {
          sbase[k] = xoff[seg * NB2MAX + bin];
          scap[k]  = total;
          if (c[k]) g[k] = atomicAdd(&rescur[seg * NB2MAX + bin], c[k]);
        } else {
          skip[k] = true;
        }
      }
      csum += c[k];
    }
  }
  uint32_t st = block_exclusive_scan<BT>(csum, 0u, SumOp(), s_scan, (uint32_t*)nullptr);
  bool spilled = false;
#pragma unroll
  for (int k = 0; k < BPT; ++k) {
    const uint32_t bin = tid * BPT + k;
    if (bin < (uint32_t)NB) {
      if (c[k] && !skip[k] && g[k] + c[k] > scap[k]) spilled = true;
      s_cnt[bin]   = st;
      s_delta[bin] = sbase[k] + g[k] - st;
      s_limit[bin] = sbase[k] + scap[k];
      st += c[k];
    }
  }
  if (spilled) {
    if (LVL == 0) hf.fail = 1;
    else if (LVL == 1) {
      if (!__hip_atomic_load(&hy.overflow, __ATOMIC_RELAXED, __HIP_MEMORY_SCOPE_AGENT)) atomicExch(&hy.overflow, 1);
    } else atomicExch(&hy.bad, 2);
  }
  __syncthreads();
#pragma unroll
  for (int j = 0; j < KPT; ++j) {
    if (j * BT + (int)tid < nvalid) {
      if constexpr (RANK16) {
        const uint32_t d = dig(to_sortable<KeyT, KIND>(key[j], desc_mask));
        s_keys[s_cnt[d] + ((packed[j >> 1] >> (16 * (j & 1))) & 0xFFFFu)] = key[j];
      } else {
        s_keys[s_cnt[packed[j] >> 16] + (packed[j] & 0xFFFFu)] = key[j];
      }
    }
  }
  __syncthreads();
  auto write_all = [&](auto&& digf) {
#pragma unroll
    for (int j = 0; j < KPT; ++j) {
      const int i = j * BT + (int)tid;
      if (i < nvalid) {
        const KeyT k       = s_keys[i];
        const uint32_t d   = digf(to_sortable<KeyT, KIND>(k, desc_mask));
        const uint32_t dst = s_delta[d] + (uint32_t)i;
        if (dst < s_limit[d]) out[dst] = k;
      }
    }
  };
  if (split) write_all(spdig); else write_all(dig);
}

constexpr int SP_KPT  = 14;
constexpr int SP_TILE = BT * SP_KPT;
constexpr size_t sp_level0_lds() { return (size_t)SP_TILE * 8 + (size_t)(3 * BINS + 16 + 4) * 4 + (size_t)2 * NW * 8 + (size_t)BINS * 8 + (size_t)SP_NLUT * 2 + (size_t)SP_TILE; }
template <int KIND, int F2>
__global__ void __launch_bounds__(BT, 4) k_sp_level0(const uint64_t* __restrict__ in, uint64_t* __restrict__ out, uint64_t desc_mask, SortPlan* plan, int64_t n)
{
  constexpr int KPT = SP_KPT, TILE = SP_TILE;
  extern __shared__ __attribute__((aligned(16))) char smem[];
  uint64_t* s_keys  = reinterpret_cast<uint64_t*>(smem);
  uint32_t* s_cnt   = reinterpret_cast<uint32_t*>(smem + (size_t)TILE * 8);
  uint32_t* s_delta = s_cnt + BINS;
  uint32_t* s_limit = s_delta + BINS;
  uint32_t* s_scan  = s_limit + BINS;
  uint32_t* s_misc  = s_scan + 16;
  unsigned long long* s_red = reinterpret_cast<unsigned long long*>(s_misc + 4);
  unsigned long long* s_tab = s_red + 2 * NW;
  uint16_t* s_lut   = reinterpret_cast<uint16_t*>(s_tab + BINS);
  uint8_t* s_bid    = reinterpret_cast<uint8_t*>(s_lut + SP_NLUT);
  HybridPlan& hy      = plan->hy;
  FastPlan& hf        = plan->hf;
  const SplitPlan& sp = plan->sp;
  if (hf.state != 1 || !sp.on || !hf.slots_ready) return;
  if ((sp.lut_log == 2u) != (F2 == 1)) return;
  const unsigned tid = threadIdx.x;
  const int64_t v    = xcd_swizzle((int64_t)blockIdx.x, (int64_t)gridDim.x);
  const int64_t per  = (int64_t)gridDim.x / NRANGE;
  const uint32_t seg = (per > 0 && v / per < NRANGE - 1) ? (uint32_t)(v / per) : (uint32_t)(NRANGE - 1);
  const int64_t base = v * TILE;
  const int nvalid   = (int)(n - base < (int64_t)TILE ? n - base : (int64_t)TILE);
  uint64_t key[KPT];
  if (nvalid == TILE) {
#pragma unroll
    for (int j = 0; j < KPT; ++j) key[j] = in[base + j * BT + (int)tid];
  } else {
#pragma unroll
    for (int j = 0; j < KPT; ++j) {
      const int idx = j * BT + (int)tid;
      key[j]        = in[base + (idx < nvalid ? idx : 0)];
    }
  }
  for (int b = tid; b < BINS; b += BT) {
    s_cnt[b] = 0;
    s_tab[b] = sp.tab[b];
  }
  for (int i = tid; i < SP_NLUT; i += BT) s_lut[i] = sp.lut[i];
  if constexpr (KIND == K_FTOTAL) {
    bool unclean = false;
#pragma unroll
    for (int j = 0; j < KPT; ++j) unclean |= float_unclean<uint64_t>(key[j]);
    if (unclean) hf.fail = 1;
  }
  {
    auto mform = [&](uint64_t k) -> uint64_t {
      if constexpr (KIND == K_FTOTAL) return to_sortable<uint64_t, KIND>(k, 0ull);
      else return k;
    };
    uint64_t vor = mform(key[0]), vnor = ~mform(key[0]);
#pragma unroll
    for (int j = 1; j < KPT; ++j) {
      vor |= mform(key[j]);
      vnor |= ~mform(key[j]);
    }
    const unsigned long long wo = wave_reduce((unsigned long long)vor, [](unsigned long long x, unsigned long long y) { return x | y; });
    const unsigned long long wn = wave_reduce((unsigned long long)vnor, [](unsigned long long x, unsigned long long y) { return x | y; });
    if (lane_id() == 0) {
      s_red[tid / GX_WAVE]      = wo;
      s_red[NW + tid / GX_WAVE] = wn;
    }
  }
  __syncthreads();
  if (tid == 0) {
    unsigned long long o = 0, no = 0;
    for (int k = 0; k < NW; ++k) {
      o |= s_red[k];
      no |= s_red[NW + k];
    }
    if (o & ~__hip_atomic_load(&hy.or_mask, __ATOMIC_RELAXED, __HIP_MEMORY_SCOPE_AGENT)) atomicOr(&hy.or_mask, o);
    if (no & ~__hip_atomic_load(&hy.nor_mask, __ATOMIC_RELAXED, __HIP_MEMORY_SCOPE_AGENT)) atomicOr(&hy.nor_mask, no);
  }
  const uint32_t nsp = sp.nsp, lut_log = sp.lut_log, lshift = sp.lshift;
  const unsigned long long kmin = sp.kmin;
  const SpLutF lf               = sp_lutf_of(sp);
  uint32_t packed[KPT];
#pragma unroll
  for (int j = 0; j < KPT; ++j) packed[j] = 0;
  const uint32_t steps = sp.lut_steps;
  if (steps <= 4u) {
#pragma unroll
    for (int j = 0; j < KPT; ++j) {
      const uint64_t k = to_sortable<uint64_t, KIND>(key[j], desc_mask);
      packed[j]        = (uint32_t)s_lut[sp_lut_cell_k<KIND, F2>(k, kmin, lut_log, lshift, lf)] & 0x1FFu;
    }
    for (uint32_t st = 0; st < steps; ++st) {
#pragma unroll
      for (int j = 0; j < KPT; ++j) {
        const uint64_t k  = to_sortable<uint64_t, KIND>(key[j], desc_mask);
        const uint32_t bb = packed[j];
        packed[j]         = bb + ((bb < nsp && s_tab[bb] <= k) ? 1u : 0u);
      }
    }
#pragma unroll
    for (int j = 0; j < KPT; ++j) {
      const bool live  = j * BT + (int)tid < nvalid;
      const uint32_t d = packed[j];
      const uint32_t r = lds_rank(s_cnt, d, live);
      packed[j]        = (d << 16) | r;
    }
  } else {
#pragma unroll
    for (int j = 0; j < KPT; ++j) {
      const bool live  = j * BT + (int)tid < nvalid;
      const uint64_t k = to_sortable<uint64_t, KIND>(key[j], desc_mask);
      const uint32_t d = sp_bucket<KIND, F2>(s_tab, s_lut, k, nsp, kmin, lut_log, lshift, lf);
      const uint32_t r = lds_rank(s_cnt, d, live);
      packed[j]        = (d << 16) | r;
    }
  }
  __syncthreads();
  uint32_t c = 0, g = 0, sbase = 0, scap = 0;
  if (tid < (unsigned)BINS) {
    c     = s_cnt[tid];
    sbase = hf.slot0[seg][tid];
    scap  = hf.cap0[seg][tid];
    if (c) g = atomicAdd(&hf.cur0[seg][tid], c);
  }
  uint32_t st = block_exclusive_scan<BT>(c, 0u, SumOp(), s_scan, (uint32_t*)nullptr);
  if (tid < (unsigned)BINS) {
    if (c && g + c > scap) hf.fail = 1;
    s_cnt[tid]   = st;
    s_delta[tid] = sbase + g - st;
    s_limit[tid] = sbase + scap;
  }
  __syncthreads();
#pragma unroll
  for (int j = 0; j < KPT; ++j) {
    if (j * BT + (int)tid < nvalid) {
      const uint32_t d   = packed[j] >> 16;
      const uint32_t pos = s_cnt[d] + (packed[j] & 0xFFFFu);
      s_keys[pos]        = key[j];
      s_bid[pos]         = (uint8_t)d;
    }
  }
  __syncthreads();
#pragma unroll
  for (int j = 0; j < KPT; ++j) {
    const int i = j * BT + (int)tid;
    if (i < nvalid) {
      const uint32_t d   = s_bid[i];
      const uint32_t dst = s_delta[d] + (uint32_t)i;
      if (dst < s_limit[d]) out[dst] = s_keys[i];
    }
  }
}

static thread_local int g_algorithm = 0;
static thread_local int g_order_mode = 0;

struct Profile {
  bool enabled = false;
  bool created = false;
  int level    = 1;
  int npass    = 0;
  hipEvent_t ev[2 * MAX_PASSES + 2];
  hipEvent_t hev[5];
  bool hybrid_marked = false;
};
constexpr int PROF_SLOTS = 64;
static thread_local Profile g_profs[PROF_SLOTS];
static thread_local int g_prof_slot = 0;
#define g_prof g_profs[g_prof_slot]
static inline void prof_mark(int idx, hipStream_t s)
{
  if (g_prof.enabled && g_prof.level == 1) (void)hipEventRecord(g_prof.ev[idx], s);
}
static inline void prof_mark_h(int idx, hipStream_t s)
{
  if (g_prof.enabled && (g_prof.level == 1 || idx <= 1)) (void)hipEventRecord(g_prof.hev[idx], s);
}
static thread_local int g_hybrid = 1;
static thread_local int g_lbw    = 16;
static thread_local int g_msd_kpt = 16;

template <typename KeyT>
constexpr int kpt_for(bool has_val)
{
  return (sizeof(KeyT) == 8 && has_val) ? 10 : 16;
}

template <typename KeyT, bool HAS_VAL, int KPT>
constexpr size_t pass_lds_bytes()
{
  return (size_t)BT * KPT * sizeof(KeyT) + (HAS_VAL ? (size_t)BT * KPT * 4 : 0) +
         (size_t)(NW * BINS + BINS + 16 + 4) * 4;
}

struct HybridCfg {
  bool on;
  int cl2;
  int bits2;
  int kpt;
  int cl2_alt;
};
static thread_local int g_cell = 0;
static inline unsigned local_sort_grid(int cells) { return (unsigned)(cells < 4096 ? cells : 4096); }
static thread_local int g_place_grid = 0;
static inline unsigned local_place_grid(int cells) { return (unsigned)((g_place_grid > 0 && g_place_grid < cells) ? g_place_grid : cells); }
template <typename KeyT, int KIND, bool HAS_VAL>
static HybridCfg hybrid_cfg(int64_t n, bool iota_payload, int algo)
{
  HybridCfg c{false, 14, 8, HAS_VAL ? 10 : g_msd_kpt, 0};
  if (sizeof(KeyT) != 8 || (HAS_VAL && !iota_payload) || algo != 0 || !g_hybrid || n < (1ll << 22)) return c;
  const bool small_ok = KIND != K_FLOAT;
  c.cl2 = (small_ok && g_cell != 16384 && (double)n / (double)(1 << 17) <= 0.955 * 8192.0) ? 13 : 14;
  if (g_cell == 8192 && small_ok) c.cl2 = 13;
  const double cell = (double)(1 << c.cl2);
  const int maxb2   = small_ok ? 9 : 8;
  int B = 9;
  while (B < 8 + maxb2 && (double)n / (double)(1ull << B) > 0.955 * cell) ++B;
  if ((double)n / (double)(1ull << B) > 0.97 * cell) return c;
  c.bits2 = B - 8;
  c.on    = true;
  if (HAS_VAL && c.cl2 == 13 && g_cell == 0) c.cl2_alt = 14;
  return c;
}

struct FastCfg {
  bool on;
  int bits2;
  int bits2_max;
  int stride;
  size_t slot_rows;
};
static thread_local int g_soft_fault      = 0;
static thread_local int g_spin_ms         = 0;
static thread_local long long g_inject_tile = -1;
static thread_local int g_cursor          = 1;
static thread_local int g_counting        = 1;
static thread_local int g_float_cursor    = 1;
static thread_local int g_split           = 1;
static thread_local int g_exp             = 0;
static thread_local float g_cursor_margin = 8.0f;
template <typename KeyT, int KIND, bool HAS_VAL>
static FastCfg fast_cfg(int64_t n, int algo, bool hybrid_on)
{
  FastCfg f{false, 9, 9, 32, 0};
  if ((sizeof(KeyT) != 8 && sizeof(KeyT) != 4) || HAS_VAL || (KIND == K_FLOAT && (sizeof(KeyT) != 8 || !g_float_cursor)) || algo != 0 || !g_cursor || n < (1ll << 25)) return f;
  if (sizeof(KeyT) == 8 ? !hybrid_on : !g_hybrid) return f;
  int B = 9;
  while (B < 18 && (double)n / (double)(1ull << B) > 0.955 * 8192.0) ++B;
  if ((double)n / (double)(1ull << B) > 0.97 * 8192.0) return f;
  f.bits2  = B - 8;
  f.bits2_max = f.bits2 < 10 ? f.bits2 + 1 : 10;
  f.stride = n >= (1ll << 27) ? 32 : 8;
  const double m   = g_cursor_margin > 0 ? g_cursor_margin : 0.0;
  const double dev = m * 1.25 * f.stride * __builtin_sqrt((double)(NRANGE * BINS) * ((double)n / f.stride + 2.0 * NRANGE * BINS));
  f.slot_rows      = (size_t)((double)n * 1.002 + dev) + (size_t)(NRANGE * BINS) * (size_t)(2 * f.stride * HF_CHUNK + 64 + 16) + 65536;
  f.on             = true;
  return f;
}

template <typename KeyT, int KIND, bool HAS_VAL>
int sort_impl(const void* keys_in, void* keys_out, const int32_t* vals_in, int32_t* vals_out, int64_t n,
              int descending, bool radix_nan_rule, void* tmp, size_t* tmp_bytes, hipStream_t stream)
{
  constexpr int KPT   = kpt_for<KeyT>(HAS_VAL);
  constexpr int TILE  = BT * KPT;
  constexpr int NPASS = sizeof(KeyT);
  if (n < 0 || tmp_bytes == nullptr) return GX_EINVAL;
  if (n > 0x7FFFFFFFll) return GX_EINVAL;
  const int64_t ntiles = n > 0 ? div_up(n, TILE) : 0;
  const int algo       = g_algorithm;

  Carver c(tmp);
  SortPlan* plan             = c.take<SortPlan>(1);
  unsigned long long* status = nullptr;
  uint32_t* tile_hist        = nullptr;
  uint32_t* partials         = nullptr;
  HybridCfg hc     = hybrid_cfg<KeyT, KIND, HAS_VAL>(n, vals_in == nullptr, algo);
  const FastCfg fc = fast_cfg<KeyT, KIND, HAS_VAL>(n, algo, hc.on);
  const size_t fc_cells = fc.on ? (size_t)n + (size_t)n / 16 + ((size_t)BINS << fc.bits2_max) * cell_slack(1 << 13) + 65536 : 0;
  if (fc.on && hc.on && hc.cl2 == 14 && (((size_t)BINS << hc.bits2) << 14) > fc_cells + (size_t)n / 4) hc.on = false;
  const bool try_hybrid = hc.on;
  const int hyb_kpt     = hc.kpt;
  const int nb1         = hc.bits2 > 8 ? NB9 : BINS;
  uint32_t* base1 = c.take<uint32_t>((size_t)NRANGE * NB2MAX);
  const bool cells = try_hybrid || fc.on;
  uint32_t* hist2 = cells ? c.take<uint32_t>((size_t)4 * BINS * NB2MAX) : nullptr;
  uint32_t* base2 = cells ? hist2 + BINS * NB2MAX : nullptr;
  uint32_t* xoff  = cells ? hist2 + 2 * BINS * NB2MAX : nullptr;
  uint32_t* todo  = cells ? c.take<uint32_t>((size_t)BINS * NB2MAX) : nullptr;
  uint32_t* biglist = fc.on ? c.take<uint32_t>((size_t)2 * BIG_LIST) : nullptr;
  const int64_t msd_tile     = (int64_t)BT * hyb_kpt;
  const int64_t msd_ntiles   = n > 0 ? div_up(n, msd_tile) : 0;
  const int64_t status_tiles = (msd_ntiles > ntiles ? msd_ntiles : ntiles) + BINS + 2 * NRANGE;
  const size_t status_words  = (size_t)status_tiles * (try_hybrid ? nb1 : BINS);
  if (algo != 1) {
    status = c.take<unsigned long long>(status_words);
  } else {
    tile_hist = c.take<uint32_t>((size_t)ntiles * BINS);
    partials  = c.take<uint32_t>(scan::partials_count(ntiles * BINS));
  }
  size_t padded = try_hybrid ? ((size_t)BINS << hc.bits2) << (hc.cl2_alt ? hc.cl2_alt : hc.cl2) : 0;
  if (fc_cells > padded) padded = fc_cells;
  const size_t nb_buf = padded > (size_t)n ? padded : (size_t)n;
  KeyT* kb_scratch = c.take<KeyT>(nb_buf);
  KeyT* slot0_buf  = fc.on ? c.take<KeyT>(fc.slot_rows) : nullptr;
  KeyT* ka_scratch = keys_out ? nullptr : c.take<KeyT>((size_t)n);
  uint32_t* vb     = HAS_VAL ? c.take<uint32_t>(nb_buf) : nullptr;
  if (tmp == nullptr) {
    *tmp_bytes = c.total();
    return 0;
  }
  if (*tmp_bytes < c.total()) return GX_ETMP;
  if (n > 0 && (keys_in == nullptr || (HAS_VAL && vals_out == nullptr))) return GX_EINVAL;
  if (n > 0 && keys_in == keys_out) return GX_EINVAL;

  GX_HIP_TRY(hipMemsetAsync(plan, 0, sizeof(SortPlan), stream));
  if (n == 0) return 0;
  Device dev;
  GX_HIP_TRY(device(&dev));
  if (algo != 1 && !fc.on) GX_HIP_TRY(hipMemsetAsync(status, 0, status_words * sizeof(unsigned long long), stream));
  if (cells) GX_HIP_TRY(hipMemsetAsync(hist2, 0, (size_t)4 * BINS * NB2MAX * sizeof(uint32_t), stream));
  const int64_t range_rows = try_hybrid ? div_up(msd_ntiles, NRANGE) * msd_tile : div_up(ntiles, NRANGE) * TILE;

  const KeyT desc_mask = descending ? KeyT(~KeyT(0)) : KeyT(0);
  g_prof.npass = NPASS;
  int64_t hblocks = div_up(n, (int64_t)BT * 8);
  if (hblocks > 2048) hblocks = 2048;
  hblocks = div_up(hblocks, NRANGE) * NRANGE;
  prof_mark(0, stream);
  g_prof.hybrid_marked = false;
  bool cursor_marked = false;
  constexpr int CK = (KIND == K_FLOAT) ? (int)K_FTOTAL : KIND;
  if constexpr ((sizeof(KeyT) == 8 || sizeof(KeyT) == 4) && !HAS_VAL && (KIND != K_FLOAT || sizeof(KeyT) == 8)) {
    if (fc.on) {
      constexpr int FT = BT * hf_kpt<KeyT>();
      constexpr int MIN_SHIFT2 = 8;
      constexpr int WORD_BYTES = (int)sizeof(typename PlaceWord<KeyT, CK, HAS_VAL>::type);
      const int64_t ftiles  = div_up(n, (int64_t)FT);
      const int64_t frange  = (ftiles / NRANGE) * FT;
      auto lds_hf = [&](int nb) { return (size_t)FT * sizeof(KeyT) + (size_t)(3 * nb + 16 + 4) * 4 + (size_t)2 * NW * 8; };
      typedef void (*HfK)(const KeyT*, KeyT*, KeyT, SortPlan*, uint32_t*, uint32_t, int64_t, KeyT*);
      HfK kf0 = k_hf_scatter<KeyT, CK, 0, 8>;
      HfK kf1 = fc.bits2_max <= 8 ? (HfK)k_hf_scatter<KeyT, CK, 1, 8> : (fc.bits2_max == 9 ? (HfK)k_hf_scatter<KeyT, CK, 1, 9> : (HfK)k_hf_scatter<KeyT, CK, 1, 10>);
      HfK kf2 = fc.bits2_max <= 8 ? (HfK)k_hf_scatter<KeyT, CK, 2, 8> : (fc.bits2_max == 9 ? (HfK)k_hf_scatter<KeyT, CK, 2, 9> : (HfK)k_hf_scatter<KeyT, CK, 2, 10>);
      const int nbf = fc.bits2_max <= 8 ? 256 : (1 << fc.bits2_max);
      const int64_t step = (int64_t)fc.stride * HF_CHUNK;
      int64_t sblocks    = div_up(div_up(n, step), (int64_t)4 * 4);
      if (sblocks > 2048) sblocks = 2048;
      const KeyT* kin = static_cast<const KeyT*>(keys_in);
      KeyT* bufA      = keys_out ? static_cast<KeyT*>(keys_out) : ka_scratch;
      hipLaunchKernelGGL((k_hf_sample<KeyT, CK, false>), dim3((unsigned)sblocks), dim3(256), 0, stream, kin, n, desc_mask, plan, fc.stride, frange);
      hipLaunchKernelGGL(k_hf_plan, dim3(1), dim3(BINS), 0, stream, plan, 0, (int)(8 * sizeof(KeyT)), n, fc.bits2, 1 << 13, fc.stride, frange, FT,
                         (unsigned long long)fc.slot_rows, g_cursor_margin, MIN_SHIFT2, fc.bits2_max, 0ull, CK == K_SIGNED ? 1 : 0, (KIND == K_FLOAT) ? 0 : g_counting);
      {
        GX_HIP_TRY(launch_lds(dev, (k_cs_count<KeyT, CK>), dim3(256), dim3(CS_BT), (size_t)4 << CS_MAXBITS, stream, kin, n, desc_mask, plan, hist2));
        hipLaunchKernelGGL(k_cs_scan, dim3(1), dim3(CS_BT), 0, stream, plan, (const uint32_t*)hist2, base2, xoff, n, NPASS);
        hipLaunchKernelGGL((k_cs_fill<KeyT, CK>), dim3(4096), dim3(256), 0, stream, bufA, n, desc_mask, (const SortPlan*)plan, (const uint32_t*)base2,
                           (const uint32_t*)xoff);
      }
      hipLaunchKernelGGL((k_hf_sample<KeyT, CK, true>), dim3((unsigned)sblocks), dim3(256), 0, stream, kin, n, desc_mask, plan, fc.stride, frange);
      const int allow_split = (sizeof(KeyT) == 8 && g_split) ? 1 : 0;
      hipLaunchKernelGGL(k_hf_plan, dim3(1), dim3(BINS), 0, stream, plan, 1, (int)(8 * sizeof(KeyT)), n, fc.bits2, 1 << 13, fc.stride, frange, FT,
                         (unsigned long long)fc.slot_rows, g_cursor_margin, MIN_SHIFT2, fc.bits2_max, 0ull, 0, 0, allow_split);
      int64_t ftiles_s = 0;
      if constexpr (sizeof(KeyT) == 8) {
        if (allow_split) {
          ftiles_s               = div_up(n, (int64_t)SP_TILE);
          const int64_t frange_s = (ftiles_s / NRANGE) * SP_TILE;
          GX_HIP_TRY(launch_lds(dev, (k_sp_plan<CK>), dim3(1), dim3(1024), (size_t)SP_NSAMP * 8, stream, kin, n, (uint64_t)desc_mask, plan, fc.bits2_max));
          hipLaunchKernelGGL((k_sp_sample<CK>), dim3((unsigned)(sblocks > 1024 ? 1024 : sblocks)), dim3(256), 0, stream, kin, n, (uint64_t)desc_mask, plan, fc.stride, frange_s);
          hipLaunchKernelGGL(k_hf_plan, dim3(1), dim3(BINS), 0, stream, plan, 1, (int)(8 * sizeof(KeyT)), n, fc.bits2, 1 << 13, fc.stride, frange_s, FT,
                             (unsigned long long)fc.slot_rows, g_cursor_margin, MIN_SHIFT2, fc.bits2_max, 0ull, 0, 0, allow_split);
        }
      }
      prof_mark(1, stream);
      prof_mark_h(0, stream);
      GX_HIP_TRY(launch_lds(dev, kf0, dim3((unsigned)ftiles), dim3(BT), lds_hf(256), stream, kin, slot0_buf, desc_mask, plan, hist2, 1u << 13, n, (KeyT*)nullptr));
      if constexpr (sizeof(KeyT) == 8) {
        if (allow_split)
        {
          GX_HIP_TRY(launch_lds(dev, (k_sp_level0<CK, 0>), dim3((unsigned)ftiles_s), dim3(BT), sp_level0_lds(), stream, kin, slot0_buf, (uint64_t)desc_mask, plan, n));
          GX_HIP_TRY(launch_lds(dev, (k_sp_level0<CK, 1>), dim3((unsigned)ftiles_s), dim3(BT), sp_level0_lds(), stream, kin, slot0_buf, (uint64_t)desc_mask, plan, n));
        }
      }
      hipLaunchKernelGGL(k_hf_plan, dim3(1), dim3(BINS), 0, stream, plan, 2, (int)(8 * sizeof(KeyT)), n, fc.bits2, 1 << 13, fc.stride, frange, FT,
                         (unsigned long long)fc.slot_rows, g_cursor_margin, MIN_SHIFT2, fc.bits2_max, (unsigned long long)nb_buf);
      prof_mark_h(1, stream);
      GX_HIP_TRY(launch_lds(dev, kf1, dim3((unsigned)(ftiles + NRANGE * BINS)), dim3(BT), lds_hf(nbf), stream, slot0_buf, kb_scratch, desc_mask, plan, hist2, 1u << 13, n, bufA));
      prof_mark_h(2, stream);
      hipLaunchKernelGGL(k_plan2, dim3(BINS), dim3(GX_WAVE), 0, stream, plan, hist2, base2, NPASS, 1);
      prof_mark_h(3, stream);
      if constexpr (sizeof(KeyT) == 8) {
        if (allow_split)
          hipLaunchKernelGGL((k_sp_fill<CK>), dim3(BINS, SP_FILL_Y), dim3(256), 0, stream, bufA, (uint64_t)desc_mask, (const SortPlan*)plan, (const uint32_t*)base2);
      }
      GX_HIP_TRY(launch_lds(dev, (k_local_place<KeyT, CK, HAS_VAL, 13>), dim3(local_place_grid(BINS << fc.bits2)), dim3((1 << 13) / 16),
                                 place_lds_bytes(13, WORD_BYTES), stream, kb_scratch, bufA, (const uint32_t*)nullptr, (uint32_t*)nullptr, desc_mask, plan, hist2,
                                 base2, todo, g_exp, 1));
      GX_HIP_TRY(launch_lds(dev, (k_local_sort<uint64_t, CK, HAS_VAL, 13, KeyT>), dim3(local_sort_grid(BINS << fc.bits2_max)), dim3((1 << 13) / 16),
                                 ((size_t)8 << 13) + (size_t)(((1 << 13) / 16 / GX_WAVE) * BINS + 32 + 2 * BINS) * 4, stream, (const KeyT*)kb_scratch, bufA,
                                 (const uint32_t*)nullptr, (uint32_t*)nullptr, (uint64_t)desc_mask, plan, hist2, base2, g_exp, 1, (const uint32_t*)todo));
      prof_mark_h(4, stream);
      g_prof.hybrid_marked = g_prof.enabled;
      cursor_marked        = true;
      hipLaunchKernelGGL(k_big_plan, dim3(1), dim3(BINS), 0, stream, plan, (unsigned long long)(fc.slot_rows / 2));
      hipLaunchKernelGGL(k_big_cells, dim3(BINS), dim3(GX_WAVE), 0, stream, (const SortPlan*)plan, (const uint32_t*)hist2, xoff, biglist);
      GX_HIP_TRY(launch_lds(dev, kf2, dim3((unsigned)(ftiles + NRANGE * BINS)), dim3(BT), lds_hf(nbf), stream, slot0_buf, kb_scratch, desc_mask, plan, hist2, 1u << 13, n, bufA));
      hipLaunchKernelGGL(k_hf_clear_status, dim3(2048), dim3(256), 0, stream, plan, reinterpret_cast<uint4*>(status), status_words / 2);
    }
  }
  if constexpr (sizeof(KeyT) == 8) {
    if (try_hybrid) {
      constexpr size_t pay   = HAS_VAL ? 4 : 0;
      constexpr bool STABLE  = KIND == K_FLOAT || HAS_VAL;
      constexpr bool SMALLOK = KIND != K_FLOAT;
      constexpr int SKPT     = HAS_VAL ? 10 : 16;
      auto lds_msd = [&](int kpt, int nb) {
        const int wrows = STABLE ? ((HAS_VAL && nb == NB9) ? NW / 2 : NW) : 2;
        return (size_t)BT * kpt * (sizeof(KeyT) + pay) + (size_t)(wrows * nb + 2 * nb + 16 + 4) * 4;
      };
      auto lds_loc = [&](int cl2) { return ((size_t)sizeof(KeyT) << cl2) + (size_t)(((1 << cl2) / 16 / GX_WAVE) * BINS + 32 + 2 * BINS) * 4; };
      typedef void (*MsdK)(MsdArgs);
      MsdK kmsd0 = HAS_VAL ? (MsdK)k_msd_pass<KeyT, KIND, HAS_VAL, 10, 4, 8>
                           : (hyb_kpt == 8 ? (MsdK)k_msd_pass<KeyT, KIND, HAS_VAL, 8, 4, 8>
                                           : (hyb_kpt == 12 ? (MsdK)k_msd_pass<KeyT, KIND, HAS_VAL, 12, 4, 8> : (MsdK)k_msd_pass<KeyT, KIND, HAS_VAL, 16, 4, 8>));
      MsdK kmsd1 = kmsd0;
      auto kloc  = k_local_sort<KeyT, KIND, HAS_VAL, 14>;
      int ls_bt  = (1 << 14) / 16;
      int kpt1 = hyb_kpt;
      if constexpr (SMALLOK) {
        if (hc.bits2 > 8) {
          kmsd1 = (MsdK)k_msd_pass<KeyT, KIND, HAS_VAL, SKPT, 4, 9>;
          kpt1  = SKPT;
        }
        if constexpr (!HAS_VAL) if (g_lbw != 4 && hyb_kpt == 16) {
          kmsd0 = g_lbw == 8 ? (MsdK)k_msd_pass<KeyT, KIND, HAS_VAL, 16, 8, 8> : (MsdK)k_msd_pass<KeyT, KIND, HAS_VAL, 16, 16, 8>;
          if (hc.bits2 > 8) kmsd1 = g_lbw == 8 ? (MsdK)k_msd_pass<KeyT, KIND, HAS_VAL, 16, 8, 9> : (MsdK)k_msd_pass<KeyT, KIND, HAS_VAL, 16, 16, 9>;
          else kmsd1 = kmsd0;
        }
        if (hc.cl2 == 13) {
          kloc  = k_local_sort<KeyT, KIND, HAS_VAL, 13>;
          ls_bt = (1 << 13) / 16;
        }
      }
      if (kpt1 != hyb_kpt) return GX_EINTERNAL;
      hipLaunchKernelGGL((k_hy_hist<KeyT, KIND, true>), dim3((unsigned)hblocks), dim3(BT), 0, stream,
                         static_cast<const KeyT*>(keys_in), n, desc_mask, plan, range_rows);
      hipLaunchKernelGGL(k_hy_plan, dim3(1), dim3(BINS), 0, stream, plan, 0, (int)(8 * sizeof(KeyT)), n, hc.bits2, 1 << hc.cl2,
                         HAS_VAL ? hc.cl2 : 0, range_rows, (int)msd_tile, base1, 0, KIND == K_SIGNED ? 1 : 0);
      hipLaunchKernelGGL((k_hy_hist<KeyT, KIND, false>), dim3((unsigned)hblocks), dim3(BT), 0, stream,
                         static_cast<const KeyT*>(keys_in), n, desc_mask, plan, range_rows);
      hipLaunchKernelGGL(k_hy_plan, dim3(1), dim3(BINS), 0, stream, plan, 1, (int)(8 * sizeof(KeyT)), n, hc.bits2, 1 << hc.cl2,
                         HAS_VAL ? hc.cl2 : 0, range_rows, (int)msd_tile, base1, hc.cl2_alt ? (1 << hc.cl2_alt) : 0);
      if (!cursor_marked) prof_mark(1, stream);
      KeyT* bufA = keys_out ? static_cast<KeyT*>(keys_out) : ka_scratch;
      KeyT* bufB = kb_scratch;
      uint32_t* valA = reinterpret_cast<uint32_t*>(vals_out);
      uint32_t* valB = vb;
      MsdArgs m;
      m.vin  = nullptr;
      m.vout = valA;
      m.plan      = plan;
      m.status    = status;
      m.n         = n;
      m.desc_mask = (uint64_t)desc_mask;
      m.in        = keys_in;
      m.out       = bufA;
      m.base      = base1;
      m.level     = 0;
      m.exp       = ((HAS_VAL && keys_out == nullptr) ? 64 : 0) | (g_exp & 32);
      m.cellcount = hist2;
      m.cellcap   = 1u << hc.cl2;
      m.spin_ticks  = (unsigned long long)g_spin_ms * 100000ull | (g_soft_fault ? SPIN_SOFT_BIT : 0ull);
      m.inject_tile = g_inject_tile;
      if (!cursor_marked) prof_mark_h(0, stream);
      GX_HIP_TRY(launch_lds(dev, kmsd0, dim3((unsigned)(msd_ntiles + NRANGE)), dim3(BT), lds_msd(hyb_kpt, BINS), stream, m));
      if (!cursor_marked) prof_mark_h(1, stream);
      m.in    = bufA;
      m.out   = bufB;
      m.vin   = valA;
      m.vout  = valB;
      m.level = 1;
      GX_HIP_TRY(launch_lds(dev, kmsd1, dim3((unsigned)(msd_ntiles + BINS + NRANGE)), dim3(BT), lds_msd(hyb_kpt, nb1), stream, m));
      if (!cursor_marked) prof_mark_h(2, stream);
      hipLaunchKernelGGL(k_plan2, dim3(BINS), dim3(GX_WAVE), 0, stream, plan, hist2, base2, NPASS, 0);
      if (!cursor_marked) prof_mark_h(3, stream);
      auto kplace = k_local_place<KeyT, KIND, HAS_VAL, 14>;
      if constexpr (SMALLOK) {
        if (hc.cl2 == 13) kplace = k_local_place<KeyT, KIND, HAS_VAL, 13>;
      }
      GX_HIP_TRY(launch_lds(dev, kplace, dim3(local_place_grid(BINS << hc.bits2)), dim3(ls_bt), place_lds_bytes(hc.cl2), stream, (const KeyT*)bufB, bufA,
                                 (const uint32_t*)valB, valA, desc_mask, plan, hist2, base2, todo, m.exp, 0));
      GX_HIP_TRY(launch_lds(dev, kloc, dim3(local_sort_grid(BINS << hc.bits2)), dim3(ls_bt), lds_loc(hc.cl2), stream, bufB, bufA, valB, valA, desc_mask,
                                 plan, hist2, base2, m.exp, 0, (const uint32_t*)todo));
      if (hc.cl2_alt == 14) {
        GX_HIP_TRY(launch_lds(dev, (k_local_place<KeyT, KIND, HAS_VAL, 14>), dim3(local_place_grid(BINS << hc.bits2)), dim3((1 << 14) / 16), place_lds_bytes(14), stream,
                                   (const KeyT*)bufB, bufA, (const uint32_t*)valB, valA, desc_mask, plan, hist2, base2, todo, m.exp, 0));
        GX_HIP_TRY(launch_lds(dev, (k_local_sort<KeyT, KIND, HAS_VAL, 14>), dim3(local_sort_grid(BINS << hc.bits2)), dim3((1 << 14) / 16), lds_loc(14), stream, bufB, bufA,
                                   valB, valA, desc_mask, plan, hist2, base2, m.exp, 0, (const uint32_t*)todo));
      }
      if (!cursor_marked) prof_mark_h(4, stream);
      if (!cursor_marked) g_prof.hybrid_marked = g_prof.enabled;
    }
  }
  hipLaunchKernelGGL((k_hist_all<KeyT, KIND>), dim3((unsigned)hblocks), dim3(BT), 0, stream,
                     static_cast<const KeyT*>(keys_in), n, desc_mask, plan, range_rows, (const KeyT*)kb_scratch);
  hipLaunchKernelGGL(k_plan, dim3(1), dim3(BINS), 0, stream, plan, NPASS, n, KIND == K_SIGNED ? 1 : 0);
  if (!try_hybrid && !cursor_marked) prof_mark(1, stream);

  PassArgs a;
  a.kbuf[0]   = const_cast<void*>(keys_in);
  a.kbuf[1]   = keys_out ? keys_out : static_cast<void*>(ka_scratch);
  a.kbuf[2]   = kb_scratch;
  a.kbufB[0]  = kb_scratch;
  a.kbufB[1]  = slot0_buf;
  a.kbufB[2]  = slot0_buf ? slot0_buf + fc.slot_rows / 2 : nullptr;
  a.vbuf[0]   = reinterpret_cast<uint32_t*>(const_cast<int32_t*>(vals_in));
  a.vbuf[1]   = reinterpret_cast<uint32_t*>(vals_out);
  a.vbuf[2]   = vb;
  a.plan      = plan;
  a.status    = status;
  a.tile_off  = tile_hist;
  a.n         = n;
  a.ntiles    = ntiles;
  a.desc_mask = (uint64_t)desc_mask;
  a.order_mode = g_order_mode;
  a.spin_ticks  = (unsigned long long)g_spin_ms * 100000ull | (g_soft_fault ? SPIN_SOFT_BIT : 0ull);
  a.inject_tile = g_inject_tile;

  constexpr size_t lds = pass_lds_bytes<KeyT, HAS_VAL, KPT>();
  auto kern_lb         = (algo == 2) ? k_radix_pass<KeyT, KIND, HAS_VAL, KPT, 1>
                                       : (cells ? k_radix_pass<KeyT, KIND, HAS_VAL, KPT, 4, true> : k_radix_pass<KeyT, KIND, HAS_VAL, KPT, 4>);
  auto kern_pre        = k_radix_pass<KeyT, KIND, HAS_VAL, KPT, 0>;
  for (int pass = 0; pass < NPASS; ++pass) {
    a.pass = pass;
    prof_mark(2 + 2 * pass, stream);
    if (algo != 1) {
      const int64_t lb_grid = (cells && algo != 2) ? div_up(ntiles, PASS_TPB) : ntiles;
      GX_HIP_TRY(launch_lds(dev, kern_lb, dim3((unsigned)lb_grid), dim3(BT), lds, stream, a));
    } else {
      hipLaunchKernelGGL((k_tile_hist<KeyT, KIND, KPT>), dim3((unsigned)ntiles), dim3(BT), 0, stream, a, tile_hist);
      scan::PlainLoader<uint32_t, uint32_t> ld{tile_hist, nullptr, 0u};
      int rc = scan::device_scan<uint32_t, uint32_t>(ld, ntiles * BINS, 0u, SumOp(), false, tile_hist, partials,
                                                     stream, &plan->pass_skip[pass]);
      if (rc) return rc;
      GX_HIP_TRY(launch_lds(dev, kern_pre, dim3((unsigned)ntiles), dim3(BT), lds, stream, a));
    }
    prof_mark(3 + 2 * pass, stream);
  }
  {
    int64_t blocks = div_up(n, 256 * 8);
    if (blocks > 4096) blocks = 4096;
    hipLaunchKernelGGL((k_finalize_copy<KeyT, HAS_VAL>), dim3((unsigned)blocks), dim3(256), 0, stream, a);
    if (fc.on)
      hipLaunchKernelGGL((k_big_distribute<KeyT>), dim3(2048), dim3(256), 0, stream, plan, (const KeyT*)slot0_buf,
                         keys_out ? static_cast<KeyT*>(keys_out) : ka_scratch, (const uint32_t*)biglist, (const uint32_t*)base2);
    if (KIND == K_FLOAT && descending && radix_nan_rule && sizeof(KeyT) >= 4) {
      hipLaunchKernelGGL((k_reverse_nan_block<KeyT, HAS_VAL>), dim3(256), dim3(256), 0, stream,
                         static_cast<KeyT*>(a.kbuf[1]), a.vbuf[1], n);
    }
  }
  GX_LAUNCH_CHECK();
  return 0;
}


struct SortxCfg {
  int bits2, bits2_max, stride;
  size_t slot_rows;
};
static inline SortxCfg sortx_cfg(int64_t n)
{
  SortxCfg f{1, 2, 8, 0};
  int B = 9;
  while (B < 18 && (double)n / (double)(1ull << B) > 0.955 * 8192.0) ++B;
  f.bits2     = B - 8;
  f.bits2_max = f.bits2 < 10 ? f.bits2 + 1 : 10;
  f.stride    = n >= (1ll << 27) ? 32 : 8;
  const double dev = 8.0 * 1.25 * f.stride * __builtin_sqrt((double)(NRANGE * BINS) * ((double)n / f.stride + 2.0 * NRANGE * BINS));
  f.slot_rows = (size_t)((double)n * 1.002 + dev) + (size_t)(NRANGE * BINS) * (size_t)(2 * f.stride * HF_CHUNK + 64 + 16) + 65536;
  return f;
}
constexpr int SORTX_MAXREG = BINS * 16 * NRANGE;

__global__ void __launch_bounds__(BINS) k_hfx_plan(SortPlan* plan, long long n, int bits2, int bits2_max, int cell_max, int min_shift2, int tile_rows,
                                                   unsigned long long or_mask, unsigned long long nor_mask, uint32_t nreg,
                                                   const uint32_t* __restrict__ breg0, uint32_t* __restrict__ x_tile0,
                                                   const uint32_t* __restrict__ x_start, const uint32_t* __restrict__ x_count,
                                                   const uint32_t* __restrict__ x_bucket, unsigned long long cell_budget)
{
  __shared__ uint32_t s_tmp[BINS / GX_WAVE + 1];
  HybridPlan& hy = plan->hy;
  FastPlan& hf   = plan->hf;
  const int t    = threadIdx.x;
  const unsigned long long V = or_mask & nor_mask;
  const int top    = V ? 63 - __builtin_clzll(V) : 0;
  const int shift0 = top - 7;
  uint32_t c = 0, tiles = 0;
  for (uint32_t q = breg0[t]; q < breg0[t + 1]; ++q) {
    c += x_count[q];
    tiles += (x_count[q] + (uint32_t)tile_rows - 1) / (uint32_t)tile_rows;
  }
  uint32_t total, ttotal;
  const uint32_t exc = block_exclusive_scan<BINS>(c, 0u, SumOp(), s_tmp, &total);
  uint32_t trun      = block_exclusive_scan<BINS>(tiles, 0u, SumOp(), s_tmp, &ttotal);
  const uint32_t fit = (uint32_t)(0.97 * (double)cell_max);
  int b2             = bits2;
  const int more     = __syncthreads_count(((unsigned long long)c >> bits2) > (unsigned long long)fit ? 1 : 0) >= 4;
  if (more && b2 < bits2_max && shift0 - b2 - 1 >= min_shift2) ++b2;
  const int shift2 = shift0 - b2;
  if (V == 0 || shift2 < min_shift2 || (long long)total != n) return;
  hy.hist0[t] = c;
  hy.gbin0[t] = exc;
  plan_cell_slots(hy, c, b2, cell_max, s_tmp, cell_budget);
  for (uint32_t q = breg0[t]; q < breg0[t + 1]; ++q) {
    x_tile0[q] = trun;
    trun += (x_count[q] + (uint32_t)tile_rows - 1) / (uint32_t)tile_rows;
  }
  if (t == 0) {
    x_tile0[nreg] = ttotal;
    hy.attempt  = 1;
    hy.shift0   = shift0;
    hy.bits2    = b2;
    hy.shift2   = shift2;
    hy.cell_max = cell_max;
    hy.or_mask  = or_mask;
    hy.nor_mask = nor_mask;
    plan_local_digits(hy, V, shift2);
    hy.fold     = 0;
    hf.ext      = 1;
    hf.nreg     = nreg;
    hf.x_tile0  = x_tile0;
    hf.x_start  = x_start;
    hf.x_count  = x_count;
    hf.x_bucket = x_bucket;
    __threadfence();
    hf.state = 3;
  }
}

template <typename KeyT>
struct SortxLayout {
  SortPlan* plan;
  uint32_t *hist2, *base2, *xoff, *todo, *biglist;
  unsigned long long* status;
  size_t status_words;
  KeyT *cells, *level0;
  size_t cells_rows, level0_rows;
  uint32_t *x_tile0, *x_start, *x_count, *x_bucket, *breg0;
  size_t total;
};
template <typename KeyT>
static SortxLayout<KeyT> sortx_layout(void* tmp, int64_t n, int64_t recv_rows_max)
{
  SortxLayout<KeyT> L{};
  Carver c(tmp);
  const SortxCfg cs = sortx_cfg(n), cr = sortx_cfg(recv_rows_max);
  L.plan          = c.take<SortPlan>(1);
  L.hist2         = c.take<uint32_t>((size_t)4 * BINS * NB2MAX);
  L.base2         = L.hist2 ? L.hist2 + BINS * NB2MAX : nullptr;
  L.xoff          = L.hist2 ? L.hist2 + 2 * BINS * NB2MAX : nullptr;
  L.todo          = c.take<uint32_t>((size_t)BINS * NB2MAX);
  L.biglist       = c.take<uint32_t>((size_t)2 * BIG_LIST);
  L.level0_rows   = cs.slot_rows + (size_t)recv_rows_max + 65536;
  L.cells_rows    = (size_t)recv_rows_max + (size_t)recv_rows_max / 16 + ((size_t)BINS << cr.bits2_max) * cell_slack(1 << 13) + 65536;
  const size_t xt = L.level0_rows / 2 / (size_t)(BT * 16) + BINS + 2 * NRANGE;
  L.status_words  = xt * BINS;
  L.status        = c.take<unsigned long long>(L.status_words);
  L.cells         = c.take<KeyT>(L.cells_rows);
  L.level0        = c.take<KeyT>(L.level0_rows);
  L.x_tile0       = c.take<uint32_t>((size_t)SORTX_MAXREG + 1);
  L.x_start       = c.take<uint32_t>((size_t)SORTX_MAXREG);
  L.x_count       = c.take<uint32_t>((size_t)SORTX_MAXREG);
  L.x_bucket      = c.take<uint32_t>((size_t)SORTX_MAXREG);
  L.breg0         = c.take<uint32_t>((size_t)BINS + 1);
  L.total         = c.total();
  return L;
}

template <typename KeyT, int KIND>
int sortx_sample(const void* keys, int64_t n, int64_t recv_rows_max, void* tmp, size_t* tmp_bytes, hipStream_t stream)
{
  auto L = sortx_layout<KeyT>(tmp, n, recv_rows_max);
  if (!tmp) {
    *tmp_bytes = L.total;
    return 0;
  }
  if (*tmp_bytes < L.total) return GX_ETMP;
  const SortxCfg cs = sortx_cfg(n);
  GX_HIP_TRY(hipMemsetAsync(L.plan, 0, sizeof(SortPlan), stream));
  GX_HIP_TRY(hipMemsetAsync(L.hist2, 0, (size_t)4 * BINS * NB2MAX * sizeof(uint32_t), stream));
  if (n == 0) return 0;
  constexpr int FT      = BT * hf_kpt<KeyT>();
  const int64_t ftiles  = div_up(n, (int64_t)FT);
  const int64_t frange  = (ftiles / NRANGE) * FT;
  const int64_t step    = (int64_t)cs.stride * HF_CHUNK;
  int64_t sblocks       = div_up(div_up(n, step), (int64_t)4 * 4);
  if (sblocks > 2048) sblocks = 2048;
  hipLaunchKernelGGL((k_hf_sample<KeyT, KIND, false>), dim3((unsigned)sblocks), dim3(256), 0, stream, static_cast<const KeyT*>(keys), n, KeyT(0), L.plan, cs.stride, frange);
  GX_LAUNCH_CHECK();
  return 0;
}

template <typename KeyT, int KIND>
int sortx_level0(const void* keys, int64_t n, int64_t recv_rows_max, const unsigned long long* masks2_host, int bits2_hint, void* tmp, hipStream_t stream)
{
  auto L = sortx_layout<KeyT>(tmp, n, recv_rows_max);
  if (n == 0) return 0;
  const SortxCfg cs = sortx_cfg(n);
  constexpr int FT      = BT * hf_kpt<KeyT>();
  constexpr int MIN_SHIFT2 = 8;
  const int64_t ftiles  = div_up(n, (int64_t)FT);
  const int64_t frange  = (ftiles / NRANGE) * FT;
  const int64_t step    = (int64_t)cs.stride * HF_CHUNK;
  int64_t sblocks       = div_up(div_up(n, step), (int64_t)4 * 4);
  if (sblocks > 2048) sblocks = 2048;
  const size_t lds0 = (size_t)FT * sizeof(KeyT) + (size_t)(3 * 256 + 16 + 4) * 4 + (size_t)2 * NW * 8;
  Device dev;
  GX_HIP_TRY(device(&dev));
  GX_HIP_TRY(hipMemcpyAsync(&L.plan->hy.or_mask, masks2_host, 2 * sizeof(unsigned long long), hipMemcpyHostToDevice, stream));
  const uint32_t one = 1;
  GX_HIP_TRY(hipMemcpyAsync(&L.plan->hf.forced_masks, &one, sizeof(one), hipMemcpyHostToDevice, stream));
  GX_HIP_TRY(hipMemcpyAsync(&L.plan->hf.forced_or, masks2_host, 2 * sizeof(unsigned long long), hipMemcpyHostToDevice, stream));
  GX_HIP_TRY(hipStreamSynchronize(stream));
  const KeyT* kin = static_cast<const KeyT*>(keys);
  hipLaunchKernelGGL(k_hf_plan, dim3(1), dim3(BINS), 0, stream, L.plan, 0, (int)(8 * sizeof(KeyT)), n, bits2_hint, 1 << 13, cs.stride, frange, FT,
                     (unsigned long long)cs.slot_rows, 8.0f, MIN_SHIFT2, bits2_hint);
  hipLaunchKernelGGL((k_hf_sample<KeyT, KIND, true>), dim3((unsigned)sblocks), dim3(256), 0, stream, kin, n, KeyT(0), L.plan, cs.stride, frange);
  hipLaunchKernelGGL(k_hf_plan, dim3(1), dim3(BINS), 0, stream, L.plan, 1, (int)(8 * sizeof(KeyT)), n, bits2_hint, 1 << 13, cs.stride, frange, FT,
                     (unsigned long long)cs.slot_rows, 8.0f, MIN_SHIFT2, bits2_hint);
  GX_HIP_TRY(launch_lds(dev, (k_hf_scatter<KeyT, KIND, 0, 8>), dim3((unsigned)ftiles), dim3(BT), lds0, stream, kin, L.level0, KeyT(0), L.plan, L.hist2, 1u << 13, n, (KeyT*)nullptr));
  hipLaunchKernelGGL(k_hf_plan, dim3(1), dim3(BINS), 0, stream, L.plan, 2, (int)(8 * sizeof(KeyT)), n, bits2_hint, 1 << 13, cs.stride, frange, FT,
                     (unsigned long long)cs.slot_rows, 8.0f, MIN_SHIFT2, bits2_hint);
  GX_LAUNCH_CHECK();
  return 0;
}

template <typename KeyT, int KIND>
int sortx_finish(int64_t n_send, int64_t recv_rows_max, int64_t n, const unsigned long long* masks2_host, const uint32_t* reg_start_host,
                 const uint32_t* reg_count_host, const uint32_t* reg_bucket_host, int nreg, void* out, void* tmp, hipStream_t stream)
{
  auto L = sortx_layout<KeyT>(tmp, n_send, recv_rows_max);
  if (nreg < 0 || nreg > SORTX_MAXREG || n > recv_rows_max + n_send) return GX_EINVAL;
  GX_HIP_TRY(hipMemsetAsync(L.plan, 0, sizeof(SortPlan), stream));
  GX_HIP_TRY(hipMemsetAsync(L.hist2, 0, (size_t)4 * BINS * NB2MAX * sizeof(uint32_t), stream));
  if (n == 0) return 0;
  const SortxCfg cr = sortx_cfg(n), cmax = sortx_cfg(recv_rows_max);
  if (cr.bits2_max > cmax.bits2_max) return GX_EINVAL;
  std::vector<uint32_t> breg0(BINS + 1, 0);
  for (int q = 0; q < nreg; ++q) {
    if (reg_bucket_host[q] >= (uint32_t)BINS || (q > 0 && reg_bucket_host[q] < reg_bucket_host[q - 1])) return GX_EINVAL;
    ++breg0[reg_bucket_host[q] + 1];
  }
  for (int b = 0; b < BINS; ++b) breg0[b + 1] += breg0[b];
  GX_HIP_TRY(hipMemcpyAsync(L.x_start, reg_start_host, sizeof(uint32_t) * nreg, hipMemcpyHostToDevice, stream));
  GX_HIP_TRY(hipMemcpyAsync(L.x_count, reg_count_host, sizeof(uint32_t) * nreg, hipMemcpyHostToDevice, stream));
  GX_HIP_TRY(hipMemcpyAsync(L.x_bucket, reg_bucket_host, sizeof(uint32_t) * nreg, hipMemcpyHostToDevice, stream));
  GX_HIP_TRY(hipMemcpyAsync(L.breg0, breg0.data(), sizeof(uint32_t) * (BINS + 1), hipMemcpyHostToDevice, stream));
  GX_HIP_TRY(hipStreamSynchronize(stream));
  constexpr int FT         = BT * hf_kpt<KeyT>();
  constexpr int MIN_SHIFT2 = 8;
  constexpr int WORD_BYTES = (int)sizeof(typename PlaceWord<KeyT, KIND, false>::type);
  auto lds_hf = [&](int nb) { return (size_t)FT * sizeof(KeyT) + (size_t)(3 * nb + 16 + 4) * 4 + (size_t)2 * NW * 8; };
  typedef void (*HfK)(const KeyT*, KeyT*, KeyT, SortPlan*, uint32_t*, uint32_t, int64_t, KeyT*);
  HfK kf1 = cr.bits2_max <= 8 ? (HfK)k_hf_scatter<KeyT, KIND, 1, 8> : (cr.bits2_max == 9 ? (HfK)k_hf_scatter<KeyT, KIND, 1, 9> : (HfK)k_hf_scatter<KeyT, KIND, 1, 10>);
  HfK kf2 = cr.bits2_max <= 8 ? (HfK)k_hf_scatter<KeyT, KIND, 2, 8> : (cr.bits2_max == 9 ? (HfK)k_hf_scatter<KeyT, KIND, 2, 9> : (HfK)k_hf_scatter<KeyT, KIND, 2, 10>);
  const int nbf = cr.bits2_max <= 8 ? 256 : (1 << cr.bits2_max);
  const size_t lds_ls = ((size_t)8 << 13) + (size_t)(((1 << 13) / 16 / GX_WAVE) * BINS + 32 + 2 * BINS) * 4;
  constexpr int KPT_L = kpt_for<KeyT>(false);
  constexpr size_t lds_pass = pass_lds_bytes<KeyT, false, KPT_L>();
  Device dev;
  GX_HIP_TRY(device(&dev));
  const int64_t l1_grid = div_up(n, (int64_t)FT) + nreg;
  KeyT* bufA = static_cast<KeyT*>(out);
  hipLaunchKernelGGL(k_hfx_plan, dim3(1), dim3(BINS), 0, stream, L.plan, (long long)n, cr.bits2, cr.bits2_max, 1 << 13, MIN_SHIFT2, FT, masks2_host[0], masks2_host[1],
                     (uint32_t)nreg, (const uint32_t*)L.breg0, L.x_tile0, (const uint32_t*)L.x_start, (const uint32_t*)L.x_count, (const uint32_t*)L.x_bucket,
                     (unsigned long long)L.cells_rows);
  GX_HIP_TRY(launch_lds(dev, kf1, dim3((unsigned)l1_grid), dim3(BT), lds_hf(nbf), stream, (const KeyT*)L.level0, L.cells, KeyT(0), L.plan, L.hist2, 1u << 13, n, (KeyT*)nullptr));
  hipLaunchKernelGGL(k_plan2, dim3(BINS), dim3(GX_WAVE), 0, stream, L.plan, L.hist2, L.base2, (int)sizeof(KeyT), 1);
  GX_HIP_TRY(launch_lds(dev, (k_local_place<KeyT, KIND, false, 13>), dim3(local_place_grid(BINS << cr.bits2)), dim3((1 << 13) / 16), place_lds_bytes(13, WORD_BYTES), stream,
                             (const KeyT*)L.cells, bufA, (const uint32_t*)nullptr, (uint32_t*)nullptr, KeyT(0), L.plan, L.hist2, L.base2, L.todo, 0, 1));
  GX_HIP_TRY(launch_lds(dev, (k_local_sort<uint64_t, KIND, false, 13, KeyT>), dim3(local_sort_grid(BINS << cr.bits2_max)), dim3((1 << 13) / 16), lds_ls, stream,
                             (const KeyT*)L.cells, bufA, (const uint32_t*)nullptr, (uint32_t*)nullptr, (uint64_t)0, L.plan, L.hist2, L.base2, 0, 1, (const uint32_t*)L.todo));
  const size_t xcap = L.level0_rows / 2;
  hipLaunchKernelGGL(k_big_plan, dim3(1), dim3(BINS), 0, stream, L.plan, (unsigned long long)xcap);
  hipLaunchKernelGGL(k_big_cells, dim3(BINS), dim3(GX_WAVE), 0, stream, (const SortPlan*)L.plan, (const uint32_t*)L.hist2, L.xoff, L.biglist);
  GX_HIP_TRY(launch_lds(dev, kf2, dim3((unsigned)l1_grid), dim3(BT), lds_hf(nbf), stream, (const KeyT*)L.level0, L.cells, KeyT(0), L.plan, L.hist2, 1u << 13, n, (KeyT*)nullptr));
  hipLaunchKernelGGL(k_hf_clear_status, dim3(2048), dim3(256), 0, stream, L.plan, reinterpret_cast<uint4*>(L.status), L.status_words / 2);
  int64_t hblocks = div_up(n, (int64_t)BT * 8);
  if (hblocks > 2048) hblocks = 2048;
  hblocks = div_up(hblocks, NRANGE) * NRANGE;
  hipLaunchKernelGGL((k_hist_all<KeyT, KIND>), dim3((unsigned)hblocks), dim3(BT), 0, stream, (const KeyT*)L.cells, (int64_t)0, KeyT(0), L.plan, (int64_t)0, (const KeyT*)L.cells);
  hipLaunchKernelGGL(k_plan, dim3(1), dim3(BINS), 0, stream, L.plan, (int)sizeof(KeyT), (int64_t)0, KIND == K_SIGNED ? 1 : 0);
  PassArgs a{};
  a.kbuf[0] = a.kbuf[1] = a.kbuf[2] = L.cells;
  a.kbufB[0] = L.cells;
  a.kbufB[1] = L.level0;
  a.kbufB[2] = L.level0 + xcap;
  a.plan      = L.plan;
  a.status    = L.status;
  a.n         = 0;
  a.ntiles    = 0;
  a.desc_mask = 0;
  const int64_t xtiles = div_up((int64_t)(n < (int64_t)xcap ? n : (int64_t)xcap), (int64_t)(BT * KPT_L));
  for (int pass = 0; pass < (int)sizeof(KeyT); ++pass) {
    a.pass = pass;
    GX_HIP_TRY(launch_lds(dev, (k_radix_pass<KeyT, KIND, false, KPT_L, 4, true>), dim3((unsigned)div_up(xtiles, (int64_t)PASS_TPB)), dim3(BT), lds_pass, stream, a));
  }
  hipLaunchKernelGGL((k_finalize_copy<KeyT, false>), dim3(1024), dim3(256), 0, stream, a);
  hipLaunchKernelGGL((k_big_distribute<KeyT>), dim3(2048), dim3(256), 0, stream, (const SortPlan*)L.plan, (const KeyT*)L.level0, bufA, (const uint32_t*)L.biglist,
                     (const uint32_t*)L.base2);
  GX_LAUNCH_CHECK();
  return 0;
}

template <bool HAS_VAL>
int dispatch(int dtype, const void* keys_in, void* keys_out, const int32_t* vals_in, int32_t* vals_out,
             int64_t n, int descending, bool radix_nan_rule, void* tmp, size_t* tmp_bytes, hipStream_t s)
{
  switch (dtype) {
    case GX_INT8: return sort_impl<uint8_t, K_SIGNED, HAS_VAL>(keys_in, keys_out, vals_in, vals_out, n, descending, radix_nan_rule, tmp, tmp_bytes, s);
    case GX_BOOL8:
    case GX_UINT8: return sort_impl<uint8_t, K_UNSIGNED, HAS_VAL>(keys_in, keys_out, vals_in, vals_out, n, descending, radix_nan_rule, tmp, tmp_bytes, s);
    case GX_INT16: return sort_impl<uint16_t, K_SIGNED, HAS_VAL>(keys_in, keys_out, vals_in, vals_out, n, descending, radix_nan_rule, tmp, tmp_bytes, s);
    case GX_UINT16: return sort_impl<uint16_t, K_UNSIGNED, HAS_VAL>(keys_in, keys_out, vals_in, vals_out, n, descending, radix_nan_rule, tmp, tmp_bytes, s);
    case GX_INT32: return sort_impl<uint32_t, K_SIGNED, HAS_VAL>(keys_in, keys_out, vals_in, vals_out, n, descending, radix_nan_rule, tmp, tmp_bytes, s);
    case GX_UINT32: return sort_impl<uint32_t, K_UNSIGNED, HAS_VAL>(keys_in, keys_out, vals_in, vals_out, n, descending, radix_nan_rule, tmp, tmp_bytes, s);
    case GX_FLOAT32: return sort_impl<uint32_t, K_FLOAT, HAS_VAL>(keys_in, keys_out, vals_in, vals_out, n, descending, radix_nan_rule, tmp, tmp_bytes, s);
    case GX_INT64: return sort_impl<uint64_t, K_SIGNED, HAS_VAL>(keys_in, keys_out, vals_in, vals_out, n, descending, radix_nan_rule, tmp, tmp_bytes, s);
    case GX_UINT64: return sort_impl<uint64_t, K_UNSIGNED, HAS_VAL>(keys_in, keys_out, vals_in, vals_out, n, descending, radix_nan_rule, tmp, tmp_bytes, s);
    case GX_FLOAT64: return sort_impl<uint64_t, K_FLOAT, HAS_VAL>(keys_in, keys_out, vals_in, vals_out, n, descending, radix_nan_rule, tmp, tmp_bytes, s);
    default: return GX_EDTYPE;
  }
}


struct BitLoader {
  const uint32_t* valid;
  __device__ __forceinline__ uint32_t operator()(int64_t i) const { return bit_is_set(valid, i) ? 1u : 0u; }
};

template <typename ElemT>
__global__ void __launch_bounds__(256) k_split_by_validity(const ElemT* __restrict__ keys,
                                                           const uint32_t* __restrict__ valid,
                                                           const uint32_t* __restrict__ pos, int64_t n,
                                                           ElemT* dense_keys, int32_t* dense_idx, int32_t* null_idx)
{
  const int64_t stride = (int64_t)gridDim.x * blockDim.x;
  for (int64_t i = (int64_t)blockIdx.x * blockDim.x + threadIdx.x; i < n; i += stride) {
    const uint32_t p = pos[i];
    if (bit_is_set(valid, i)) {
      dense_keys[p] = keys[i];
      dense_idx[p]  = (int32_t)i;
    } else {
      null_idx[i - p] = (int32_t)i;
    }
  }
}

template <typename ElemT>
int sorted_order_nullable(int dtype, const void* keys, const uint32_t* valid, int64_t n, int64_t null_count,
                          int descending, int nulls_before, int32_t* out, void* tmp, size_t* tmp_bytes,
                          hipStream_t stream)
{
  const int64_t nvalid = n - null_count;
  size_t sort_bytes    = 0;
  int rc = dispatch<true>(dtype, nullptr, nullptr, nullptr, nullptr, nvalid, descending, false, nullptr,
                          &sort_bytes, stream);
  if (rc) return rc;
  Carver c(tmp);
  char* sort_tmp      = c.take<char>(sort_bytes);
  uint32_t* pos       = c.take<uint32_t>((size_t)n);
  uint32_t* partials  = c.take<uint32_t>(scan::partials_count(n));
  ElemT* dense_keys   = c.take<ElemT>((size_t)nvalid);
  int32_t* dense_idx  = c.take<int32_t>((size_t)nvalid);
  if (tmp == nullptr) {
    *tmp_bytes = c.total();
    return 0;
  }
  if (*tmp_bytes < c.total()) return GX_ETMP;
  if (n == 0) return 0;
  const bool nulls_first = (nulls_before != 0) != (descending != 0);
  rc = scan::device_scan<uint32_t, uint32_t>(BitLoader{valid}, n, 0u, SumOp(), false, pos, partials, stream);
  if (rc) return rc;
  int64_t blocks = div_up(n, 256 * 4);
  if (blocks > 4096) blocks = 4096;
  hipLaunchKernelGGL((k_split_by_validity<ElemT>), dim3((unsigned)blocks), dim3(256), 0, stream,
                     static_cast<const ElemT*>(keys), valid, pos, n, dense_keys, dense_idx,
                     out + (nulls_first ? 0 : nvalid));
  GX_LAUNCH_CHECK();
  size_t sb = sort_bytes;
  return dispatch<true>(dtype, dense_keys, nullptr, dense_idx, out + (nulls_first ? null_count : 0), nvalid,
                        descending, false, sort_tmp, &sb, stream);
}

template <typename K32, int KIND>
__global__ void __launch_bounds__(256) k_pack_words(const K32* __restrict__ keys, int64_t n, K32 desc_mask, int rbits, uint64_t* __restrict__ words)
{
  const int64_t stride = (int64_t)gridDim.x * blockDim.x;
  for (int64_t i = (int64_t)blockIdx.x * blockDim.x + threadIdx.x; i < n; i += stride)
    words[i] = ((uint64_t)to_sortable<K32, KIND>(keys[i], desc_mask) << rbits) | (uint64_t)i;
}
__global__ void __launch_bounds__(256) k_unpack_rows(const uint64_t* __restrict__ words, int64_t n, int rbits, int32_t* __restrict__ rows)
{
  const int64_t stride = (int64_t)gridDim.x * blockDim.x;
  const uint64_t rmask = (1ull << rbits) - 1ull;
  for (int64_t i = (int64_t)blockIdx.x * blockDim.x + threadIdx.x; i < n; i += stride) rows[i] = (int32_t)(uint32_t)(words[i] & rmask);
}
static thread_local int g_order_words = 0;
static inline bool order_words32_applies(int dtype, int64_t n)
{
  return g_order_words && (dtype == GX_INT32 || dtype == GX_UINT32) && n >= (1ll << 25) && g_algorithm == 0 && g_hybrid && g_cursor;
}
template <typename K32, int KIND>
int sorted_order_words32(const void* keys, int64_t n, int descending, int32_t* out, void* tmp, size_t* tmp_bytes, hipStream_t stream)
{
  size_t sort_bytes = 0;
  int rc = sort_impl<uint64_t, K_UNSIGNED, false>(nullptr, nullptr, nullptr, nullptr, n, 0, false, nullptr, &sort_bytes, stream);
  if (rc) return rc;
  Carver c(tmp);
  char* sort_tmp  = c.take<char>(sort_bytes);
  uint64_t* w_in  = c.take<uint64_t>((size_t)n);
  uint64_t* w_out = c.take<uint64_t>((size_t)n);
  if (tmp == nullptr) {
    *tmp_bytes = c.total();
    return 0;
  }
  if (*tmp_bytes < c.total()) return GX_ETMP;
  if (keys == nullptr || out == nullptr) return GX_EINVAL;
  int64_t blocks = div_up(n, 256 * 8);
  if (blocks > 8192) blocks = 8192;
  int rbits = 1;
  while (((int64_t)1 << rbits) < n) ++rbits;
  hipLaunchKernelGGL((k_pack_words<K32, KIND>), dim3((unsigned)blocks), dim3(256), 0, stream, static_cast<const K32*>(keys), n,
                     descending ? K32(~K32(0)) : K32(0), rbits, w_in);
  size_t sb = sort_bytes;
  rc = sort_impl<uint64_t, K_UNSIGNED, false>(w_in, w_out, nullptr, nullptr, n, 0, false, sort_tmp, &sb, stream);
  if (rc) return rc;
  hipLaunchKernelGGL(k_unpack_rows, dim3((unsigned)blocks), dim3(256), 0, stream, w_out, n, rbits, out);
  GX_LAUNCH_CHECK();
// ... 311 lines not shown
```

Measured before the change: 89.75 billion rows/s.

## Cap fallback kernel grids with persistent tile loops and fuse hist2 zeroing into sampling

Fallback-path kernels (MSD passes, the level-2 hf scatter, local place/sort) now launch a grid capped at a fixed number of workgroups per CU. The MSD and scatter kernels loop over tiles persistently, and the level-2 scatter exits early when its path is inactive. This is meant to cut the cost of launching huge grids of blocks that mostly return immediately. The hist2 memset is folded into the sample kernel. Sampling now gives each block a contiguous chunk range with deeper unroll, computes range membership by comparisons instead of division, and uses a count-only LDS aggregation. The risks are less parallelism on the fallback path and more complex tile-claim loops.

Measured after the change: 91.52 billion rows/s (median of 6 runs). 2.0% higher.

```diff
diff --git a/cudf_amd/csrc/gx_common.hpp b/cudf_amd/csrc/gx_common.hpp
--- a/cudf_amd/csrc/gx_common.hpp
+++ b/cudf_amd/csrc/gx_common.hpp
@@ -223,6 +223,21 @@
     return live ? atomicAdd(&counters[d], 1u) : 0u;
   }
   return live ? atomicAdd(&counters[d], 1u) : 0u;
+}
+
+__device__ __forceinline__ void lds_count(uint32_t* counters, uint32_t d, bool live)
+{
+  const uint64_t act = ballot(live);
+  if (act == 0) return;
+  const int leader    = __builtin_ctzll(act);
+  const uint32_t dl   = shfl(d, leader);
+  const uint64_t same = ballot(live && d == dl);
+  if (same == act || __builtin_popcountll(same) >= 8) {
+    if ((int)lane_id() == leader) atomicAdd(&counters[dl], (uint32_t)__builtin_popcountll(same));
+    if (live && d != dl) atomicAdd(&counters[d], 1u);
+    return;
+  }
+  if (live) atomicAdd(&counters[d], 1u);
 }
 
 struct SumOp {
diff --git a/cudf_amd/csrc/gx_sort.hip b/cudf_amd/csrc/gx_sort.hip
--- a/cudf_amd/csrc/gx_sort.hip
+++ b/cudf_amd/csrc/gx_sort.hip
@@ -876,7 +876,7 @@
 };
 
 template <typename KeyT, int KIND, bool HAS_VAL, int KPT, int LBW, int NBL>
-__global__ void __launch_bounds__(BT, (KPT <= 8 ? 8 : (KPT <= 12 ? 6 : 4))) k_msd_pass(MsdArgs a)
+__device__ __forceinline__ bool msd_pass_tile(const MsdArgs& a)
 {
   constexpr int TILE = BT * KPT;
   constexpr int NB   = 1 << NBL;
@@ -898,7 +898,7 @@
   SortPlan* plan = a.plan;
   HybridPlan& hy = plan->hy;
   const int lvl  = a.level;
-  if (!hy.attempt || plan->hf.state == 3) return;
+  if (!hy.attempt || plan->hf.state == 3) return false;
   const KeyT* kin      = static_cast<const KeyT*>(a.in);
   KeyT* kout           = static_cast<KeyT*>(a.out);
   const uint32_t* vin  = a.vin;
@@ -940,7 +940,7 @@
   }
   __syncthreads();
   const uint32_t gtile = s_misc[0];
-  if (gtile == 0xFFFFFFFFu) return;
+  if (gtile == 0xFFFFFFFFu) return false;
   const uint32_t seg   = s_misc[1];
   const uint32_t jt    = s_misc[2];
   const int64_t base   = (int64_t)hy.seg_start[lvl][seg] + (int64_t)jt * TILE;
@@ -1103,6 +1103,17 @@
         if (HAS_VAL) vout[dst] = s_vals[i];
       }
     }
+  }
+  return true;
+}
+
+template <typename KeyT, int KIND, bool HAS_VAL, int KPT, int LBW, int NBL, bool MULTI = false>
+__global__ void __launch_bounds__(BT, (KPT <= 8 ? 8 : (KPT <= 12 ? 6 : 4))) k_msd_pass(MsdArgs a)
+{
+  if constexpr (MULTI) {
+    while (msd_pass_tile<KeyT, KIND, HAS_VAL, KPT, LBW, NBL>(a)) __syncthreads();
+  } else {
+    msd_pass_tile<KeyT, KIND, HAS_VAL, KPT, LBW, NBL>(a);
   }
 }
 
@@ -1721,8 +1732,12 @@
 
 template <typename KeyT, int KIND, bool HIST>
 __global__ void __launch_bounds__(256) k_hf_sample(const KeyT* __restrict__ in, int64_t n, KeyT desc_mask, SortPlan* plan, int stride,
-                                                   int64_t range_rows)
-{
+                                                   int64_t range_rows, uint4* __restrict__ zero = nullptr, size_t zero16 = 0)
+{
+  if (!HIST && zero != nullptr) {
+    const size_t zs = (size_t)gridDim.x * 256;
+    for (size_t i = (size_t)blockIdx.x * 256 + threadIdx.x; i < zero16; i += zs) zero[i] = uint4{0u, 0u, 0u, 0u};
+  }
   HybridPlan& hy = plan->hy;
   FastPlan& hf   = plan->hf;
   if (HIST && (hf.state != 1 || hf.hist_ready)) return;
@@ -1734,20 +1749,26 @@
   const Digit0 dig      = HIST ? digit0_of(hy, (int)(8 * sizeof(KeyT))) : Digit0{(int)(8 * sizeof(KeyT) - 8), 0, 0xFFu, 0u};
   const int64_t step    = (int64_t)stride * HF_CHUNK;
   const int64_t nchunks = div_up(n, step);
-  const int64_t nw      = (int64_t)gridDim.x * 4;
-  constexpr int U       = 8;
+  const int64_t per     = div_up(nchunks, (int64_t)gridDim.x);
+  const int64_t c_lo    = (int64_t)blockIdx.x * per;
+  const int64_t c_hi    = c_lo + per < nchunks ? c_lo + per : nchunks;
+  constexpr int64_t nw  = 4;
+  constexpr int U       = 16;
+  int64_t rstart[NRANGE - 1];
+#pragma unroll
+  for (int k = 1; k < NRANGE; ++k) rstart[k - 1] = range_rows > 0 ? (int64_t)k * range_rows : (int64_t)0;
   KeyT vor = 0, vnor = 0, vfold = 0;
-  for (int64_t c0 = (int64_t)blockIdx.x * 4 + tid / GX_WAVE; c0 < nchunks; c0 += nw * U) {
+  for (int64_t c0 = c_lo + tid / GX_WAVE; c0 < c_hi; c0 += nw * U) {
     KeyT raw[U];
 #pragma unroll
     for (int u = 0; u < U; ++u) {
       const int64_t row = (c0 + u * nw) * step + lane;
-      raw[u]            = (c0 + u * nw < nchunks && row < n) ? in[row] : KeyT(0);
+      raw[u]            = (c0 + u * nw < c_hi && row < n) ? in[row] : KeyT(0);
     }
 #pragma unroll
     for (int u = 0; u < U; ++u) {
       const int64_t row = (c0 + u * nw) * step + lane;
-      const bool live   = c0 + u * nw < nchunks && row < n;
+      const bool live   = c0 + u * nw < c_hi && row < n;
       const KeyT k      = to_sortable<KeyT, KIND>(raw[u], desc_mask);
       if (!HIST && live) {
         if constexpr (KIND == K_FTOTAL) {
@@ -1757,9 +1778,10 @@
         vnor |= (KeyT)~k;
         if (KIND == K_SIGNED) vfold |= (KeyT)(raw[u] ^ (KeyT)(KeyT(0) - (KeyT)(raw[u] >> (8 * sizeof(KeyT) - 1))));
       }
-      const int64_t r64 = range_rows > 0 ? row / range_rows : (int64_t)(NRANGE - 1);
-      const int r       = r64 < NRANGE - 1 ? (int)r64 : NRANGE - 1;
-      (void)lds_rank(s_hist + r * BINS, dig(k), live);
+      int r = 0;
+#pragma unroll
+      for (int q = 1; q < NRANGE; ++q) r += row >= rstart[q - 1] ? 1 : 0;
+      lds_count(s_hist + r * BINS, dig(k), live);
     }
   }
   if (!HIST) {
@@ -2658,8 +2680,8 @@
 }
 
 template <typename KeyT, int KIND, int LVL, int NBL>
-__global__ void __launch_bounds__(BT, 4) k_hf_scatter(const KeyT* __restrict__ in, KeyT* __restrict__ out, KeyT desc_mask, SortPlan* plan,
-                                                     uint32_t* __restrict__ cellcur, uint32_t cellcap, int64_t n, KeyT* __restrict__ fin = nullptr)
+__device__ __forceinline__ void hf_scatter_tile(const KeyT* __restrict__ in, KeyT* __restrict__ out, KeyT desc_mask, SortPlan* plan,
+                                                uint32_t* __restrict__ cellcur, int64_t n, KeyT* __restrict__ fin, int64_t vblock, int64_t nblocks)
 {
   constexpr int KPT = hf_kpt<KeyT>(), TILE = BT * KPT, NB = 1 << NBL, BPT = NB > BT ? NB / BT : 1;
   extern __shared__ __attribute__((aligned(16))) char smem[];
@@ -2680,12 +2702,12 @@
   const uint32_t* xoff = cellcur + 2 * BINS * NB2MAX;
   uint32_t* rescur     = cellcur + 3 * BINS * NB2MAX;
   const unsigned tid = threadIdx.x;
-  const int64_t v    = xcd_swizzle((int64_t)blockIdx.x, (int64_t)gridDim.x);
+  const int64_t v    = xcd_swizzle(vblock, nblocks);
   int64_t base;
   int nvalid;
   uint32_t seg;
   if (LVL == 0) {
-    const int64_t per = (int64_t)gridDim.x / NRANGE;
+    const int64_t per = nblocks / NRANGE;
     seg               = (per > 0 && v / per < NRANGE - 1) ? (uint32_t)(v / per) : (uint32_t)(NRANGE - 1);
     base              = v * TILE;
     nvalid            = (int)(n - base < (int64_t)TILE ? n - base : (int64_t)TILE);
@@ -2702,8 +2724,12 @@
       }
     }
     __syncthreads();
-    const uint32_t q  = s_misc[0];
-    const uint32_t jt = s_misc[1];
+    uint32_t q  = s_misc[0];
+    uint32_t jt = s_misc[1];
+    if constexpr (LVL == 2) {
+      q  = (uint32_t)__builtin_amdgcn_readfirstlane((int)q);
+      jt = (uint32_t)__builtin_amdgcn_readfirstlane((int)jt);
+    }
     seg               = q / NRANGE;
     if (LVL == 2 && !hy.bigbucket[seg]) return;
     base              = (int64_t)hf.reg_start[q] + (int64_t)jt * TILE;
@@ -2721,8 +2747,12 @@
       }
     }
     __syncthreads();
-    const uint32_t q  = s_misc[0];
-    const uint32_t jt = s_misc[1];
+    uint32_t q  = s_misc[0];
+    uint32_t jt = s_misc[1];
+    if constexpr (LVL == 2) {
+      q  = (uint32_t)__builtin_amdgcn_readfirstlane((int)q);
+      jt = (uint32_t)__builtin_amdgcn_readfirstlane((int)jt);
+    }
     seg               = hf.x_bucket[q];
     if (LVL == 2 && !hy.bigbucket[seg]) return;
     base              = (int64_t)hf.x_start[q] + (int64_t)jt * TILE;
@@ -2922,6 +2952,22 @@
     }
   };
   if (split) write_all(spdig); else write_all(dig);
+}
+
+template <typename KeyT, int KIND, int LVL, int NBL>
+__global__ void __launch_bounds__(BT, 4) k_hf_scatter(const KeyT* __restrict__ in, KeyT* __restrict__ out, KeyT desc_mask, SortPlan* plan,
+                                                     uint32_t* __restrict__ cellcur, uint32_t cellcap, int64_t n, KeyT* __restrict__ fin = nullptr,
+                                                     uint32_t ntiles = 0)
+{
+  if constexpr (LVL == 2) {
+    if (plan->hf.state != 3 || !(plan->hy.ok && plan->hy.lsd_mode)) return;
+    for (uint32_t t = blockIdx.x; t < ntiles; t += gridDim.x) {
+      hf_scatter_tile<KeyT, KIND, LVL, NBL>(in, out, desc_mask, plan, cellcur, n, fin, (int64_t)t, (int64_t)ntiles);
+      __syncthreads();
+    }
+  } else {
+    hf_scatter_tile<KeyT, KIND, LVL, NBL>(in, out, desc_mask, plan, cellcur, n, fin, (int64_t)blockIdx.x, (int64_t)gridDim.x);
+  }
 }
 
 constexpr int SP_KPT  = 14;
@@ -3130,6 +3176,13 @@
 static inline unsigned local_sort_grid(int cells) { return (unsigned)(cells < 4096 ? cells : 4096); }
 static thread_local int g_place_grid = 0;
 static inline unsigned local_place_grid(int cells) { return (unsigned)((g_place_grid > 0 && g_place_grid < cells) ? g_place_grid : cells); }
+enum class Role { primary, fallback };
+constexpr int FALLBACK_WGS_PER_CU = 16;
+static inline unsigned role_grid(const Device& dev, Role role, int64_t want)
+{
+  const int64_t cap = (int64_t)FALLBACK_WGS_PER_CU * dev.cus;
+  return (unsigned)((role == Role::fallback && want > cap) ? cap : want);
+}
 template <typename KeyT, int KIND, bool HAS_VAL>
 static HybridCfg hybrid_cfg(int64_t n, bool iota_payload, int algo)
 {
@@ -3245,7 +3298,8 @@
   Device dev;
   GX_HIP_TRY(device(&dev));
   if (algo != 1 && !fc.on) GX_HIP_TRY(hipMemsetAsync(status, 0, status_words * sizeof(unsigned long long), stream));
-  if (cells) GX_HIP_TRY(hipMemsetAsync(hist2, 0, (size_t)4 * BINS * NB2MAX * sizeof(uint32_t), stream));
+  const size_t hist2_bytes = (size_t)4 * BINS * NB2MAX * sizeof(uint32_t);
+  if (cells && !fc.on) GX_HIP_TRY(hipMemsetAsync(hist2, 0, hist2_bytes, stream));
   const int64_t range_rows = try_hybrid ? div_up(msd_ntiles, NRANGE) * msd_tile : div_up(ntiles, NRANGE) * TILE;
 
   const KeyT desc_mask = descending ? KeyT(~KeyT(0)) : KeyT(0);
@@ -3265,7 +3319,7 @@
       const int64_t ftiles  = div_up(n, (int64_t)FT);
       const int64_t frange  = (ftiles / NRANGE) * FT;
       auto lds_hf = [&](int nb) { return (size_t)FT * sizeof(KeyT) + (size_t)(3 * nb + 16 + 4) * 4 + (size_t)2 * NW * 8; };
-      typedef void (*HfK)(const KeyT*, KeyT*, KeyT, SortPlan*, uint32_t*, uint32_t, int64_t, KeyT*);
+      typedef void (*HfK)(const KeyT*, KeyT*, KeyT, SortPlan*, uint32_t*, uint32_t, int64_t, KeyT*, uint32_t);
       HfK kf0 = k_hf_scatter<KeyT, CK, 0, 8>;
       HfK kf1 = fc.bits2_max <= 8 ? (HfK)k_hf_scatter<KeyT, CK, 1, 8> : (fc.bits2_max == 9 ? (HfK)k_hf_scatter<KeyT, CK, 1, 9> : (HfK)k_hf_scatter<KeyT, CK, 1, 10>);
       HfK kf2 = fc.bits2_max <= 8 ? (HfK)k_hf_scatter<KeyT, CK, 2, 8> : (fc.bits2_max == 9 ? (HfK)k_hf_scatter<KeyT, CK, 2, 9> : (HfK)k_hf_scatter<KeyT, CK, 2, 10>);
@@ -3275,7 +3329,8 @@
       if (sblocks > 2048) sblocks = 2048;
       const KeyT* kin = static_cast<const KeyT*>(keys_in);
       KeyT* bufA      = keys_out ? static_cast<KeyT*>(keys_out) : ka_scratch;
-      hipLaunchKernelGGL((k_hf_sample<KeyT, CK, false>), dim3((unsigned)sblocks), dim3(256), 0, stream, kin, n, desc_mask, plan, fc.stride, frange);
+      hipLaunchKernelGGL((k_hf_sample<KeyT, CK, false>), dim3((unsigned)sblocks), dim3(256), 0, stream, kin, n, desc_mask, plan, fc.stride, frange,
+                         reinterpret_cast<uint4*>(hist2), hist2_bytes / sizeof(uint4));
       hipLaunchKernelGGL(k_hf_plan, dim3(1), dim3(BINS), 0, stream, plan, 0, (int)(8 * sizeof(KeyT)), n, fc.bits2, 1 << 13, fc.stride, frange, FT,
                          (unsigned long long)fc.slot_rows, g_cursor_margin, MIN_SHIFT2, fc.bits2_max, 0ull, CK == K_SIGNED ? 1 : 0, (KIND == K_FLOAT) ? 0 : g_counting);
       {
@@ -3301,7 +3356,7 @@
       }
       prof_mark(1, stream);
       prof_mark_h(0, stream);
-      GX_HIP_TRY(launch_lds(dev, kf0, dim3((unsigned)ftiles), dim3(BT), lds_hf(256), stream, kin, slot0_buf, desc_mask, plan, hist2, 1u << 13, n, (KeyT*)nullptr));
+      GX_HIP_TRY(launch_lds(dev, kf0, dim3((unsigned)ftiles), dim3(BT), lds_hf(256), stream, kin, slot0_buf, desc_mask, plan, hist2, 1u << 13, n, (KeyT*)nullptr, 0u));
       if constexpr (sizeof(KeyT) == 8) {
         if (allow_split)
         {
@@ -3312,7 +3367,7 @@
       hipLaunchKernelGGL(k_hf_plan, dim3(1), dim3(BINS), 0, stream, plan, 2, (int)(8 * sizeof(KeyT)), n, fc.bits2, 1 << 13, fc.stride, frange, FT,
                          (unsigned long long)fc.slot_rows, g_cursor_margin, MIN_SHIFT2, fc.bits2_max, (unsigned long long)nb_buf);
       prof_mark_h(1, stream);
-      GX_HIP_TRY(launch_lds(dev, kf1, dim3((unsigned)(ftiles + NRANGE * BINS)), dim3(BT), lds_hf(nbf), stream, slot0_buf, kb_scratch, desc_mask, plan, hist2, 1u << 13, n, bufA));
+      GX_HIP_TRY(launch_lds(dev, kf1, dim3((unsigned)(ftiles + NRANGE * BINS)), dim3(BT), lds_hf(nbf), stream, slot0_buf, kb_scratch, desc_mask, plan, hist2, 1u << 13, n, bufA, 0u));
       prof_mark_h(2, stream);
       hipLaunchKernelGGL(k_plan2, dim3(BINS), dim3(GX_WAVE), 0, stream, plan, hist2, base2, NPASS, 1);
       prof_mark_h(3, stream);
@@ -3331,7 +3386,8 @@
       cursor_marked        = true;
       hipLaunchKernelGGL(k_big_plan, dim3(1), dim3(BINS), 0, stream, plan, (unsigned long long)(fc.slot_rows / 2));
       hipLaunchKernelGGL(k_big_cells, dim3(BINS), dim3(GX_WAVE), 0, stream, (const SortPlan*)plan, (const uint32_t*)hist2, xoff, biglist);
-      GX_HIP_TRY(launch_lds(dev, kf2, dim3((unsigned)(ftiles + NRANGE * BINS)), dim3(BT), lds_hf(nbf), stream, slot0_buf, kb_scratch, desc_mask, plan, hist2, 1u << 13, n, bufA));
+      GX_HIP_TRY(launch_lds(dev, kf2, dim3(role_grid(dev, Role::fallback, ftiles + NRANGE * BINS)), dim3(BT), lds_hf(nbf), stream, slot0_buf, kb_scratch, desc_mask, plan,
+                            hist2, 1u << 13, n, bufA, (uint32_t)(ftiles + NRANGE * BINS)));
       hipLaunchKernelGGL(k_hf_clear_status, dim3(2048), dim3(256), 0, stream, plan, reinterpret_cast<uint4*>(status), status_words / 2);
     }
   }
@@ -3370,6 +3426,16 @@
         }
       }
       if (kpt1 != hyb_kpt) return GX_EINTERNAL;
+      const Role lb_role = (fc.on && SMALLOK) ? Role::fallback : Role::primary;
+      bool msd_multi     = false;
+      if constexpr (!HAS_VAL && SMALLOK) {
+        if (lb_role == Role::fallback && hyb_kpt == 16 && g_lbw == 16) {
+          kmsd0 = (MsdK)k_msd_pass<KeyT, KIND, HAS_VAL, 16, 16, 8, true>;
+          kmsd1 = hc.bits2 > 8 ? (MsdK)k_msd_pass<KeyT, KIND, HAS_VAL, 16, 16, 9, true> : kmsd0;
+          msd_multi = true;
+        }
+      }
+      const Role msd_role = msd_multi ? Role::fallback : Role::primary;
       hipLaunchKernelGGL((k_hy_hist<KeyT, KIND, true>), dim3((unsigned)hblocks), dim3(BT), 0, stream,
                          static_cast<const KeyT*>(keys_in), n, desc_mask, plan, range_rows);
       hipLaunchKernelGGL(k_hy_plan, dim3(1), dim3(BINS), 0, stream, plan, 0, (int)(8 * sizeof(KeyT)), n, hc.bits2, 1 << hc.cl2,
@@ -3400,14 +3466,14 @@
       m.spin_ticks  = (unsigned long long)g_spin_ms * 100000ull | (g_soft_fault ? SPIN_SOFT_BIT : 0ull);
       m.inject_tile = g_inject_tile;
       if (!cursor_marked) prof_mark_h(0, stream);
-      GX_HIP_TRY(launch_lds(dev, kmsd0, dim3((unsigned)(msd_ntiles + NRANGE)), dim3(BT), lds_msd(hyb_kpt, BINS), stream, m));
+      GX_HIP_TRY(launch_lds(dev, kmsd0, dim3(role_grid(dev, msd_role, msd_ntiles + NRANGE)), dim3(BT), lds_msd(hyb_kpt, BINS), stream, m));
       if (!cursor_marked) prof_mark_h(1, stream);
       m.in    = bufA;
       m.out   = bufB;
       m.vin   = valA;
       m.vout  = valB;
       m.level = 1;
-      GX_HIP_TRY(launch_lds(dev, kmsd1, dim3((unsigned)(msd_ntiles + BINS + NRANGE)), dim3(BT), lds_msd(hyb_kpt, nb1), stream, m));
+      GX_HIP_TRY(launch_lds(dev, kmsd1, dim3(role_grid(dev, msd_role, msd_ntiles + BINS + NRANGE)), dim3(BT), lds_msd(hyb_kpt, nb1), stream, m));
       if (!cursor_marked) prof_mark_h(2, stream);
       hipLaunchKernelGGL(k_plan2, dim3(BINS), dim3(GX_WAVE), 0, stream, plan, hist2, base2, NPASS, 0);
       if (!cursor_marked) prof_mark_h(3, stream);
@@ -3415,14 +3481,14 @@
       if constexpr (SMALLOK) {
         if (hc.cl2 == 13) kplace = k_local_place<KeyT, KIND, HAS_VAL, 13>;
       }
-      GX_HIP_TRY(launch_lds(dev, kplace, dim3(local_place_grid(BINS << hc.bits2)), dim3(ls_bt), place_lds_bytes(hc.cl2), stream, (const KeyT*)bufB, bufA,
+      GX_HIP_TRY(launch_lds(dev, kplace, dim3(role_grid(dev, lb_role, local_place_grid(BINS << hc.bits2))), dim3(ls_bt), place_lds_bytes(hc.cl2), stream, (const KeyT*)bufB, bufA,
                                  (const uint32_t*)valB, valA, desc_mask, plan, hist2, base2, todo, m.exp, 0));
-      GX_HIP_TRY(launch_lds(dev, kloc, dim3(local_sort_grid(BINS << hc.bits2)), dim3(ls_bt), lds_loc(hc.cl2), stream, bufB, bufA, valB, valA, desc_mask,
+      GX_HIP_TRY(launch_lds(dev, kloc, dim3(role_grid(dev, lb_role, local_sort_grid(BINS << hc.bits2))), dim3(ls_bt), lds_loc(hc.cl2), stream, bufB, bufA, valB, valA, desc_mask,
                                  plan, hist2, base2, m.exp, 0, (const uint32_t*)todo));
       if (hc.cl2_alt == 14) {
-        GX_HIP_TRY(launch_lds(dev, (k_local_place<KeyT, KIND, HAS_VAL, 14>), dim3(local_place_grid(BINS << hc.bits2)), dim3((1 << 14) / 16), place_lds_bytes(14), stream,
+        GX_HIP_TRY(launch_lds(dev, (k_local_place<KeyT, KIND, HAS_VAL, 14>), dim3(role_grid(dev, lb_role, local_place_grid(BINS << hc.bits2))), dim3((1 << 14) / 16), place_lds_bytes(14), stream,
                                    (const KeyT*)bufB, bufA, (const uint32_t*)valB, valA, desc_mask, plan, hist2, base2, todo, m.exp, 0));
-        GX_HIP_TRY(launch_lds(dev, (k_local_sort<KeyT, KIND, HAS_VAL, 14>), dim3(local_sort_grid(BINS << hc.bits2)), dim3((1 << 14) / 16), lds_loc(14), stream, bufB, bufA,
+        GX_HIP_TRY(launch_lds(dev, (k_local_sort<KeyT, KIND, HAS_VAL, 14>), dim3(role_grid(dev, lb_role, local_sort_grid(BINS << hc.bits2))), dim3((1 << 14) / 16), lds_loc(14), stream, bufB, bufA,
                                    valB, valA, desc_mask, plan, hist2, base2, m.exp, 0, (const uint32_t*)todo));
       }
       if (!cursor_marked) prof_mark_h(4, stream);
@@ -3655,7 +3721,7 @@
   hipLaunchKernelGGL((k_hf_sample<KeyT, KIND, true>), dim3((unsigned)sblocks), dim3(256), 0, stream, kin, n, KeyT(0), L.plan, cs.stride, frange);
   hipLaunchKernelGGL(k_hf_plan, dim3(1), dim3(BINS), 0, stream, L.plan, 1, (int)(8 * sizeof(KeyT)), n, bits2_hint, 1 << 13, cs.stride, frange, FT,
                      (unsigned long long)cs.slot_rows, 8.0f, MIN_SHIFT2, bits2_hint);
-  GX_HIP_TRY(launch_lds(dev, (k_hf_scatter<KeyT, KIND, 0, 8>), dim3((unsigned)ftiles), dim3(BT), lds0, stream, kin, L.level0, KeyT(0), L.plan, L.hist2, 1u << 13, n, (KeyT*)nullptr));
+  GX_HIP_TRY(launch_lds(dev, (k_hf_scatter<KeyT, KIND, 0, 8>), dim3((unsigned)ftiles), dim3(BT), lds0, stream, kin, L.level0, KeyT(0), L.plan, L.hist2, 1u << 13, n, (KeyT*)nullptr, 0u));
   hipLaunchKernelGGL(k_hf_plan, dim3(1), dim3(BINS), 0, stream, L.plan, 2, (int)(8 * sizeof(KeyT)), n, bits2_hint, 1 << 13, cs.stride, frange, FT,
                      (unsigned long long)cs.slot_rows, 8.0f, MIN_SHIFT2, bits2_hint);
   GX_LAUNCH_CHECK();
@@ -3688,7 +3754,7 @@
   constexpr int MIN_SHIFT2 = 8;
   constexpr int WORD_BYTES = (int)sizeof(typename PlaceWord<KeyT, KIND, false>::type);
   auto lds_hf = [&](int nb) { return (size_t)FT * sizeof(KeyT) + (size_t)(3 * nb + 16 + 4) * 4 + (size_t)2 * NW * 8; };
-  typedef void (*HfK)(const KeyT*, KeyT*, KeyT, SortPlan*, uint32_t*, uint32_t, int64_t, KeyT*);
+  typedef void (*HfK)(const KeyT*, KeyT*, KeyT, SortPlan*, uint32_t*, uint32_t, int64_t, KeyT*, uint32_t);
   HfK kf1 = cr.bits2_max <= 8 ? (HfK)k_hf_scatter<KeyT, KIND, 1, 8> : (cr.bits2_max == 9 ? (HfK)k_hf_scatter<KeyT, KIND, 1, 9> : (HfK)k_hf_scatter<KeyT, KIND, 1, 10>);
   HfK kf2 = cr.bits2_max <= 8 ? (HfK)k_hf_scatter<KeyT, KIND, 2, 8> : (cr.bits2_max == 9 ? (HfK)k_hf_scatter<KeyT, KIND, 2, 9> : (HfK)k_hf_scatter<KeyT, KIND, 2, 10>);
   const int nbf = cr.bits2_max <= 8 ? 256 : (1 << cr.bits2_max);
@@ -3702,7 +3768,7 @@
   hipLaunchKernelGGL(k_hfx_plan, dim3(1), dim3(BINS), 0, stream, L.plan, (long long)n, cr.bits2, cr.bits2_max, 1 << 13, MIN_SHIFT2, FT, masks2_host[0], masks2_host[1],
                      (uint32_t)nreg, (const uint32_t*)L.breg0, L.x_tile0, (const uint32_t*)L.x_start, (const uint32_t*)L.x_count, (const uint32_t*)L.x_bucket,
                      (unsigned long long)L.cells_rows);
-  GX_HIP_TRY(launch_lds(dev, kf1, dim3((unsigned)l1_grid), dim3(BT), lds_hf(nbf), stream, (const KeyT*)L.level0, L.cells, KeyT(0), L.plan, L.hist2, 1u << 13, n, (KeyT*)nullptr));
+  GX_HIP_TRY(launch_lds(dev, kf1, dim3((unsigned)l1_grid), dim3(BT), lds_hf(nbf), stream, (const KeyT*)L.level0, L.cells, KeyT(0), L.plan, L.hist2, 1u << 13, n, (KeyT*)nullptr, 0u));
   hipLaunchKernelGGL(k_plan2, dim3(BINS), dim3(GX_WAVE), 0, stream, L.plan, L.hist2, L.base2, (int)sizeof(KeyT), 1);
   GX_HIP_TRY(launch_lds(dev, (k_local_place<KeyT, KIND, false, 13>), dim3(local_place_grid(BINS << cr.bits2)), dim3((1 << 13) / 16), place_lds_bytes(13, WORD_BYTES), stream,
                              (const KeyT*)L.cells, bufA, (const uint32_t*)nullptr, (uint32_t*)nullptr, KeyT(0), L.plan, L.hist2, L.base2, L.todo, 0, 1));
@@ -3711,7 +3777,8 @@
   const size_t xcap = L.level0_rows / 2;
   hipLaunchKernelGGL(k_big_plan, dim3(1), dim3(BINS), 0, stream, L.plan, (unsigned long long)xcap);
   hipLaunchKernelGGL(k_big_cells, dim3(BINS), dim3(GX_WAVE), 0, stream, (const SortPlan*)L.plan, (const uint32_t*)L.hist2, L.xoff, L.biglist);
-  GX_HIP_TRY(launch_lds(dev, kf2, dim3((unsigned)l1_grid), dim3(BT), lds_hf(nbf), stream, (const KeyT*)L.level0, L.cells, KeyT(0), L.plan, L.hist2, 1u << 13, n, (KeyT*)nullptr));
+  GX_HIP_TRY(launch_lds(dev, kf2, dim3(role_grid(dev, Role::fallback, l1_grid)), dim3(BT), lds_hf(nbf), stream, (const KeyT*)L.level0, L.cells, KeyT(0), L.plan, L.hist2, 1u << 13, n,
+                        (KeyT*)nullptr, (uint32_t)l1_grid));
   hipLaunchKernelGGL(k_hf_clear_status, dim3(2048), dim3(256), 0, stream, L.plan, reinterpret_cast<uint4*>(L.status), L.status_words / 2);
   int64_t hblocks = div_up(n, (int64_t)BT * 8);
   if (hblocks > 2048) hblocks = 2048;
```
